# gdalsanto/flamo

Hardware: AMD Instinct MI355X
Metric: freq-bin*channel products/sec (fwd+bwd), nfft=96000 8x8ch (higher is better)
Workload: dtype f32; 1 GPU; BASELINE configs[1]: Shell(FFT -> Series(Matrix 8x8, GEQ 8x8) -> iFFT), nfft=96000, batch 32 per GPU, fwd+bwd of (y**2).mean(), parameter grads; nfft=96000, channels=8, batch_per_gpu=32, parallelism=dp1 (batch), input_grad=False

## Files before the change

flamo_amd/_lib.py:

```python
from __future__ import annotations

import ctypes as C
import os
import subprocess
import threading

_HERE = os.path.dirname(os.path.abspath(__file__))
LIB_PATH = os.environ.get("FLAMO_HIP_LIB") or os.path.join(_HERE, "libflamo_hip.so")
CSRC = os.path.join(_HERE, "csrc")

_lock = threading.Lock()
_lib = None

_vp, _i, _l, _d, _sz = C.c_void_p, C.c_int, C.c_long, C.c_double, C.c_size_t

_SIGNATURES = {
    "fl_version": (_i, []),
    "fl_last_error": (C.c_char_p, []),
    "fl_twiddle_fill_f32": (_i, [_vp, _i, _vp]),
    "fl_twiddle_fill_f64": (_i, [_vp, _i, _vp]),
    "fl_fft_plan": (_i, [_i, _i, C.POINTER(_i), C.POINTER(_i)]),
    "fl_fft_scratch_elems": (_sz, [_i, _i, _i]),
    "fl_debug_set_fft_max_single": (_i, [_i]),
    "fl_debug_set_fft_fast": (_i, [_i]),
    "fl_rfft_f32": (_i, [_vp, _l, _i, _vp, _l, _vp, _vp, _i, _i, _d, _d, _i, _vp]),
    "fl_rfft_f64": (_i, [_vp, _l, _i, _vp, _l, _vp, _vp, _i, _i, _d, _d, _i, _vp]),
    "fl_rfft_ci_f32": (_i, [_vp, _i, _i, _vp, _l, _vp, _vp, _i, _i, _d, _d, _i, _vp]),
    "fl_rfft_ci_f64": (_i, [_vp, _i, _i, _vp, _l, _vp, _vp, _i, _i, _d, _d, _i, _vp]),
    "fl_irfft_f32": (_i, [_vp, _l, _vp, _l, _i, _vp, _vp, _i, _i, _d, _d, _i, _vp]),
    "fl_irfft_f64": (_i, [_vp, _l, _vp, _l, _i, _vp, _vp, _i, _i, _d, _d, _i, _vp]),
    "fl_transpose": (_i, [_vp, _vp, _i, _i, _i, _l, _i, _vp]),
    "fl_spec_plan": (_i, [_i, C.POINTER(_i), C.POINTER(_i)]),
    "fl_spec_supports": (_i, [_i, _i, _i]),
    "fl_spec_supports_f64": (_i, [_i, _i, _i]),
    "fl_spec_aux_elems": (_sz, [_i]),
    "fl_spec_aux_fill_f32": (_i, [_vp, _i, _vp]),
    "fl_spec_aux_fill_f64": (_i, [_vp, _i, _vp]),
    "fl_debug_set_spec": (_i, [_i, _i]),
    "fl_debug_set_spec_times": (_i, [_vp]),
    "fl_spec_cols_fwd_f32": (_i, [_vp, _i, _i, _i, _vp, _vp, _i, _d, _vp]),
    "fl_spec_cols_fwd_f64": (_i, [_vp, _i, _i, _i, _vp, _vp, _i, _d, _vp]),
    "fl_spec_gradh_loop_supports_f32": (_i, [_i, _i, _i]),
    "fl_spec_gradh_loop_supports_f64": (_i, [_i, _i, _i]),
    "fl_spec_gradh_loop_f32": (_i, [_vp, _vp, _l, _l, _vp, _l, _l, _vp, _i, _i, _i, _i, _d, _i, _d, _vp, _vp]),
    "fl_spec_gradh_loop_f64": (_i, [_vp, _vp, _l, _l, _vp, _l, _l, _vp, _i, _i, _i, _i, _d, _i, _d, _vp, _vp]),
    "fl_spec_mid_f32": (_i, [_vp, _vp, _vp, _l, _l, _vp, _l, _l, _i, _vp, _i, _i, _i, _i, _d, _i, _i, _vp]),
    "fl_spec_mid_f64": (_i, [_vp, _vp, _vp, _l, _l, _vp, _l, _l, _i, _vp, _i, _i, _i, _i, _d, _i, _i, _vp]),
    "fl_spec_walk_supports": (_i, [_i, _i, _i]),
    "fl_spec_walk_spectrum_elems": (_sz, [_i, _i, _i]),
    "fl_spec_walk_workgroups": (_i, [_i, _i]),
    "fl_spec_walk_partition": (_i, [_i, _i, _i, C.POINTER(_i)]),
    "fl_spec_mid_walk_f32": (_i, [_vp, _vp, _vp, _vp, _l, _l, _i, _vp, _i, _i, _i, _i, _d, _i, _i, _vp, _vp]),
    "fl_spec_gradh_slices": (_i, [_i, _i]),
    "fl_spec_gradh_walk_f32": (_i, [_vp, _vp, _vp, _l, _l, _l, _i, _vp, _i, _i, _i, _i, _d, _i, _vp, _vp]),
    "fl_sum_parts_c64": (_i, [_vp, _l, _i, _vp, _l, _vp]),
    "fl_debug_set_walk": (_i, [_i, _i, _i, _vp]),
    "fl_debug_set_walk_stamps": (_i, [_vp]),
    "fl_wall_clock_khz": (_i, []),
    "fl_spec_cols_inv_f32": (_i, [_vp, _vp, _i, _i, _i, _i, _vp, _i, _d, _d, _vp, _vp, _vp, _vp]),
    "fl_spec_cols_blocks_f32": (_i, [_i, _i, _i]),
    "fl_spec_cols_blocks_f64": (_i, [_i, _i, _i]),
    "fl_spec_cols_inv_inplace_ok_f32": (_i, [_i, _i]),
    "fl_spec_cols_inv_inplace_ok_f64": (_i, [_i, _i]),
    "fl_spec_cols_inv_grad_supported_f32": (_i, [_i, _i]),
    "fl_spec_cols_inv_grad_supported_f64": (_i, [_i, _i]),
    "fl_mean_square_final_f32": (_i, [_vp, _i, _d, _vp, _vp]),
    "fl_mean_square_final_f64": (_i, [_vp, _i, _d, _vp, _vp]),
    "fl_pack_toggle": (_i, [_vp, _i, _vp, _vp, _vp, _vp]),
    "fl_spec_cols_inv_f64": (_i, [_vp, _vp, _i, _i, _i, _i, _vp, _i, _d, _d, _vp, _vp, _vp, _vp]),
    "fl_permute_bins_c64": (_i, [_vp, _l, _vp, _l, _i, _i, _i, _vp]),
    "fl_permute_bins_c128": (_i, [_vp, _l, _vp, _l, _i, _i, _i, _vp]),
    "fl_mimo_c64": (_i, [_vp, _l, _l, _l, _i, _vp, _l, _l, _l, _vp, _l, _l, _l, _i, _i, _i, _i, _i, _vp]),
    "fl_mimo_c128": (_i, [_vp, _l, _l, _l, _i, _vp, _l, _l, _l, _vp, _l, _l, _l, _i, _i, _i, _i, _i, _vp]),
    "fl_mimo_diag_c64": (_i, [_vp, _l, _l, _i, _vp, _l, _l, _l, _vp, _l, _l, _l, _i, _i, _i, _i, _vp]),
    "fl_mimo_diag_c128": (_i, [_vp, _l, _l, _i, _vp, _l, _l, _l, _vp, _l, _l, _l, _i, _i, _i, _i, _vp]),
    "fl_mimo_gradh_c64": (_i, [_vp, _l, _l, _l, _vp, _l, _l, _l, _vp, _l, _d, _i, _i, _i, _i, _i, _vp]),
    "fl_mimo_gradh_c128": (_i, [_vp, _l, _l, _l, _vp, _l, _l, _l, _vp, _l, _d, _i, _i, _i, _i, _i, _vp]),
    "fl_mimo_gradh_scaled_c64": (_i, [_vp, _l, _l, _l, _vp, _l, _l, _l, _vp, _l, _d, _vp, _i, _i, _i, _i, _i, _vp]),
    "fl_mimo_gradh_scaled_c128": (_i, [_vp, _l, _l, _l, _vp, _l, _l, _l, _vp, _l, _d, _vp, _i, _i, _i, _i, _i, _vp]),
    "fl_mimo_gradh_diag_c64": (_i, [_vp, _l, _l, _l, _vp, _l, _l, _l, _vp, _l, _i, _i, _i, _i, _vp]),
    "fl_mimo_gradh_diag_c128": (_i, [_vp, _l, _l, _l, _vp, _l, _l, _l, _vp, _l, _i, _i, _i, _i, _vp]),
    "fl_mimo_gradw_blocks": (_i, [_i]),
    "fl_debug_set_mimo_variant": (_i, [_i, _i]),
    "fl_mimo_gradw_c64": (_i, [_vp, _l, _l, _l, _vp, _l, _l, _l, _vp, _vp, _i, _i, _i, _i, _i, _vp]),
    "fl_mimo_gradw_c128": (_i, [_vp, _l, _l, _l, _vp, _l, _l, _l, _vp, _vp, _i, _i, _i, _i, _i, _vp]),
    "fl_mimo_gradw_re_c64": (_i, [_vp, _l, _l, _l, _vp, _l, _l, _l, _vp, _vp, _i, _i, _i, _i, _i, _vp]),
    "fl_mimo_gradw_re_c128": (_i, [_vp, _l, _l, _l, _vp, _l, _l, _l, _vp, _vp, _i, _i, _i, _i, _i, _vp]),
    "fl_delay_response_c64": (_i, [_vp, _vp, _i, _vp, _i, _i, _i, _vp, _l, _vp]),
    "fl_delay_response_c128": (_i, [_vp, _vp, _i, _vp, _i, _i, _i, _vp, _l, _vp]),
    "fl_sos_response_c64": (_i, [_vp, _vp, _i, _i, _d, _vp, _i, _i, _i, _vp, _l, _vp]),
    "fl_sos_response_f32eval_c64": (_i, [_vp, _vp, _i, _i, _d, _vp, _i, _i, _i, _vp, _l, _vp]),
    "fl_sos_response_c128": (_i, [_vp, _vp, _i, _i, _d, _vp, _i, _i, _i, _vp, _l, _vp]),
    "fl_sos_bwd_blocks": (_i, [_i, _i, _i, _i]),
    "fl_debug_set_sos_chunk": (_i, [_i]),
    "fl_debug_set_rc_fast": (_i, [_i]),
    "fl_sos_response_bwd_c64": (_i, [_vp, _l, _vp, _l, _vp, _vp, _i, _i, _d, _vp, _i, _i, _i, _vp, _vp]),
    "fl_sos_response_bwd_c128": (_i, [_vp, _l, _vp, _l, _vp, _vp, _i, _i, _d, _vp, _i, _i, _i, _vp, _vp]),
    "fl_sos_response_apply_max_ni": (_i, [_i]),
    "fl_sos_response_apply_c64": (_i, [_vp, _vp, _i, _i, _i, _vp, _l, _l, _i, _d, _vp, _i, _i, _i, _vp, _l, _vp, _l, _l, _vp]),
    "fl_sos_response_bwd_outer_c64": (_i, [_vp, _l, _l, _vp, _l, _l, _i, _i, _i, _vp, _l, _vp, _vp, _i, _d, _vp, _i, _i, _i, _vp, _vp]),
    "fl_sos_response_rc_c64": (_i, [_vp, _vp, _i, _i, _i, _i, _vp, _d, _vp, _i, _i, _i, _vp, _l, _vp, _l, _i, _vp]),
    "fl_geq_response_c64": (_i, [_vp, _i, _i, _vp, _vp, _vp, _i, _d, _vp, _i, _i, _i, _vp, _l, _i, _vp]),
    "fl_geq_response_rc_c64": (_i, [_vp, _i, _i, _vp, _vp, _vp, _i, _i, _i, _vp, _d, _vp, _i, _i, _i, _vp, _l, _vp, _l, _i, _vp]),
    "fl_sos_response_bwd_rc_c64": (_i, [_vp, _l, _vp, _l, _vp, _vp, _i, _i, _i, _i, _vp, _d, _vp, _i, _i, _i, _vp, _vp, _vp]),
    "fl_geq_sections": (_i, [_vp, _i, _i, _i, _vp, _vp, _vp, _vp]),
    "fl_geq_sections_bwd": (_i, [_vp, _i, _vp, _vp, _l, _i, _i, _i, _vp, _vp, _vp]),
    "fl_geq_sections_bwd_w": (_i, [_vp, _i, _vp, _vp, _l, _i, _i, _i, _vp, _vp, _vp, _i, _i, _vp, _vp]),
    "fl_geq_sections_bwd_w64": (_i, [_vp, _i, _vp, _vp, _l, _i, _i, _i, _vp, _vp, _vp, _i, _i, _vp, _vp]),
    "fl_sos_response_rc_c128": (_i, [_vp, _vp, _i, _i, _i, _i, _vp, _d, _vp, _i, _i, _i, _vp, _l, _vp, _l, _vp]),
    "fl_geq_response_rc_c128": (_i, [_vp, _i, _i, _vp, _vp, _vp, _i, _i, _i, _vp, _d, _vp, _i, _i, _i, _vp, _l, _vp, _l, _vp]),
    "fl_sos_response_bwd_rc_c128": (_i, [_vp, _l, _vp, _l, _vp, _vp, _i, _i, _i, _i, _vp, _d, _vp, _i, _i, _i, _vp, _vp, _vp]),
    "fl_geq_bwd_lanes_blocks": (_i, [_i, _i, _i, _i, _i, _i, _i, _i]),
    "fl_geq_bwd_lanes_wrows": (_i, [_i, _i, _i, _i, _i, _i, _i]),
    "fl_geq_response_bwd_lanes_c64": (_i, [_i, _vp, _l, _vp, _l, _vp, _vp, _i, _i, _i, _i, _vp, _d, _vp, _i, _i, _i, _vp, _vp, _vp, _vp]),
    "fl_geq_sections_bwd_lanes": (_i, [_vp, _i, _vp, _vp, _i, _vp, _vp, _d, _i, _i, _vp, _vp, _vp, _i, _i, _vp, _vp]),
    "fl_geq_bwd_lanes_blocks_f64": (_i, [_i, _i, _i, _i, _i, _i, _i, _i]),
    "fl_geq_bwd_lanes_wrows_f64": (_i, [_i, _i, _i, _i, _i, _i, _i]),
    "fl_geq_response_bwd_lanes_c128": (_i, [_i, _vp, _l, _vp, _l, _vp, _vp, _i, _i, _i, _i, _vp, _d, _vp, _i, _i, _i, _vp, _vp, _vp, _vp]),
    "fl_geq_sections_bwd_lanes_f64": (_i, [_vp, _i, _vp, _vp, _i, _vp, _vp, _d, _i, _i, _vp, _vp, _vp, _i, _i, _vp, _vp]),
    "fl_debug_set_cascade_lanes": (_i, [_i, _i, _i]),
    "fl_debug_set_cascade_stamps": (_i, [_vp, _i]),
    "fl_solve_max_n": (_i, [_i]),
    "fl_solve_ws_max_n": (_i, []),
    "fl_solve_ws_bytes": (_l, [_i, _i, _i]),
    "fl_solve_ws_c64": (_i, [_vp, _l, _i, _i, _vp, _l, _l, _l, _vp, _l, _l, _l, _i, _i, _i, _i, _vp, _l, _vp]),
    "fl_solve_ws_c128": (_i, [_vp, _l, _i, _i, _vp, _l, _l, _l, _vp, _l, _l, _l, _i, _i, _i, _i, _vp, _l, _vp]),
    "fl_solve_c64": (_i, [_vp, _l, _i, _i, _vp, _l, _l, _l, _vp, _l, _l, _l, _i, _i, _i, _i, _vp]),
    "fl_solve_c128": (_i, [_vp, _l, _i, _i, _vp, _l, _l, _l, _vp, _l, _l, _l, _i, _i, _i, _i, _vp]),
    "fl_solve_scaled_c64": (_i, [_vp, _l, _vp, _l, _i, _vp, _l, _l, _l, _vp, _l, _l, _l, _i, _i, _i, _i, _vp]),
    "fl_solve_scaled_c128": (_i, [_vp, _l, _vp, _l, _i, _vp, _l, _l, _l, _vp, _l, _l, _l, _i, _i, _i, _i, _vp]),
    "fl_solve_kept_lu_elems": (_sz, [_i, _i, _i]),
    "fl_solve_kept_piv_elems": (_sz, [_i, _i, _i]),
    "fl_solve_scaled_keep_c64": (_i, [_vp, _l, _vp, _l, _vp, _l, _l, _l, _vp, _l, _l, _l, _i, _i, _i, _i, _vp, _vp, _vp]),
    "fl_solve_scaled_keep_c128": (_i, [_vp, _l, _vp, _l, _vp, _l, _l, _l, _vp, _l, _l, _l, _i, _i, _i, _i, _vp, _vp, _vp]),
    "fl_solve_kept_adjoint_c64": (_i, [_vp, _vp, _vp, _l, _l, _l, _vp, _l, _l, _l, _i, _i, _i, _i, _vp]),
    "fl_solve_kept_adjoint_c128": (_i, [_vp, _vp, _vp, _l, _l, _l, _vp, _l, _l, _l, _i, _i, _i, _i, _vp]),
    "fl_solve_fdn_keep_tile": (_i, [_i, _i]),
    "fl_solve_fdn_wadj_supported": (_i, [_i]),
    "fl_solve_dud2_grads_w_c64": (_i, [_vp, _l, _l, _vp, _l, _l, _vp, _vp, _l, _l, _vp, _l, _vp, _l, _vp, _l, _l, _l, _i, _i, _i, _vp, _l, _vp, _l,
                                       _vp, _vp, _vp, _vp, _l, _vp, _l, _vp, _vp]),
    "fl_solve_dud2_grads_w_c128": (_i, [_vp, _l, _l, _vp, _l, _l, _vp, _vp, _l, _l, _vp, _l, _vp, _l, _vp, _l, _l, _l, _i, _i, _i, _vp, _l, _vp, _l,
                                       _vp, _vp, _vp, _vp, _l, _vp, _l, _vp, _vp]),
    "fl_solve_fdn_wadj_c64": (_i, [_vp, _l, _l, _vp, _l, _l, _vp, _vp, _l, _l, _vp, _i, _vp, _l, _vp, _i, _vp, _l, _vp, _l, _l, _l, _i, _i, _i, _vp, _l, _vp]),
    "fl_solve_fdn_wadj_c128": (_i, [_vp, _l, _l, _vp, _l, _l, _vp, _vp, _l, _l, _vp, _i, _vp, _l, _vp, _i, _vp, _l, _vp, _l, _l, _l, _i, _i, _i, _vp, _l, _vp]),
    "fl_solve_fdn_keep_c64": (_i, [_vp, _l, _l, _vp, _l, _l, _vp, _vp, _l, _l, _vp, _i, _vp, _l, _vp, _i, _vp, _l, _vp, _l, _l, _l, _i, _i, _i, _vp, _vp, _vp]),
    "fl_solve_fdn_keep_c128": (_i, [_vp, _l, _l, _vp, _l, _l, _vp, _vp, _l, _l, _vp, _i, _vp, _l, _vp, _i, _vp, _l, _vp, _l, _l, _l, _i, _i, _i, _vp, _vp, _vp]),
    "fl_solve_kept_adjoint_rank1_c64": (_i, [_vp, _vp, _i, _vp, _i, _vp, _l, _vp, _l, _l, _l, _i, _i, _i, _vp]),
    "fl_solve_kept_adjoint_rank1_c128": (_i, [_vp, _vp, _i, _vp, _i, _vp, _l, _vp, _l, _l, _l, _i, _i, _i, _vp]),
    "fl_solve_dud_c64": (_i, [_vp, _l, _l, _vp, _vp, _l, _l, _i, _vp, _l, _l, _l, _vp, _l, _l, _l, _i, _i, _i, _i, _vp]),
    "fl_solve_dud_c128": (_i, [_vp, _l, _l, _vp, _vp, _l, _l, _i, _vp, _l, _l, _l, _vp, _l, _l, _l, _i, _i, _i, _i, _vp]),
    "fl_solve_dud_grads_blocks": (_i, [_i, _i]),
    "fl_solve_fdn_c64": (_i, [_vp, _l, _l, _vp, _l, _l, _vp, _vp, _l, _l, _i, _vp, _i, _vp, _l, _vp, _i, _vp, _l, _vp, _l, _l, _l, _i, _i, _i, _vp]),
    "fl_solve_fdn_c128": (_i, [_vp, _l, _l, _vp, _l, _l, _vp, _vp, _l, _l, _i, _vp, _i, _vp, _l, _vp, _i, _vp, _l, _vp, _l, _l, _l, _i, _i, _i, _vp]),
    "fl_solve_dud2_c64": (_i, [_vp, _l, _l, _vp, _l, _l, _i, _vp, _vp, _l, _l, _i, _vp, _l, _l, _l, _vp, _l, _l, _l, _i, _i, _i, _i, _vp]),
    "fl_solve_dud2_c128": (_i, [_vp, _l, _l, _vp, _l, _l, _i, _vp, _vp, _l, _l, _i, _vp, _l, _l, _l, _vp, _l, _l, _l, _i, _i, _i, _i, _vp]),
    "fl_solve_dud2_grads_c64": (_i, [_vp, _l, _l, _vp, _l, _l, _vp, _vp, _l, _l, _vp, _vp, _l, _l, _l, _i, _i, _i, _i, _vp, _l, _vp, _l, _vp, _vp, _vp, _vp, _l, _vp, _l, _vp, _vp]),
    "fl_solve_dud2_grads_c128": (_i, [_vp, _l, _l, _vp, _l, _l, _vp, _vp, _l, _l, _vp, _vp, _l, _l, _l, _i, _i, _i, _i, _vp, _l, _vp, _l, _vp, _vp, _vp, _vp, _l, _vp, _l, _vp, _vp]),
    "fl_solve_dud_grads_c64": (_i, [_vp, _l, _l, _vp, _vp, _l, _l, _vp, _vp, _l, _l, _l, _i, _i, _i, _i, _vp, _l, _vp, _l, _vp, _vp, _vp]),
    "fl_solve_dud_grads_c128": (_i, [_vp, _l, _l, _vp, _vp, _l, _l, _vp, _vp, _l, _l, _l, _i, _i, _i, _i, _vp, _l, _vp, _l, _vp, _vp, _vp]),
    "fl_debug_set_solve_variant": (_i, [_i]),
    "fl_mean_square_scratch_bytes": (_sz, []),
    "fl_mean_square_f32": (_i, [_vp, _l, _l, _l, _vp, _vp, _vp]),
    "fl_mean_square_f64": (_i, [_vp, _l, _l, _l, _vp, _vp, _vp]),
    "fl_mean_square_bwd_f32": (_i, [_vp, _vp, _vp, _l, _l, _l, _vp]),
    "fl_mean_square_bwd_f64": (_i, [_vp, _vp, _vp, _l, _l, _l, _vp]),
    "fl_cabs_c64": (_i, [_vp, _vp, _l, _l, _l, _l, _vp]),
    "fl_cabs_c128": (_i, [_vp, _vp, _l, _l, _l, _l, _vp]),
    "fl_cabs_bwd_c64": (_i, [_vp, _vp, _vp, _l, _l, _l, _l, _vp]),
    "fl_cabs_bwd_c128": (_i, [_vp, _vp, _vp, _l, _l, _l, _l, _vp]),
    "fl_sparsity_f32": (_i, [_vp, _i, _i, _vp, _vp]),
    "fl_sparsity_f64": (_i, [_vp, _i, _i, _vp, _vp]),
    "fl_sparsity_bwd_f32": (_i, [_vp, _vp, _i, _i, _vp, _vp]),
    "fl_sparsity_bwd_f64": (_i, [_vp, _vp, _i, _i, _vp, _vp]),
    "fl_mse_f32": (_i, [_vp, _vp, _l, _i, _vp, _vp, _vp]),
    "fl_mse_f64": (_i, [_vp, _vp, _l, _i, _vp, _vp, _vp]),
    "fl_mse_bwd_f32": (_i, [_vp, _vp, _vp, _vp, _l, _i, _vp]),
    "fl_mse_bwd_f64": (_i, [_vp, _vp, _vp, _vp, _l, _i, _vp]),
    "fl_matrix_exp_stash_elems": (_sz, [_i]),
    "fl_debug_set_expm_mfma": (_i, [_i]),
    "fl_matrix_exp_f32": (_i, [_vp, _i, _i, _vp, _vp, _vp]),
    "fl_matrix_exp_f64": (_i, [_vp, _i, _i, _vp, _vp, _vp]),
    "fl_matrix_exp_bwd_f32": (_i, [_vp, _i, _i, _vp, _vp, _vp]),
    "fl_matrix_exp_bwd_f64": (_i, [_vp, _i, _i, _vp, _vp, _vp]),
    "fl_matrix_exp_cplx_f32": (_i, [_vp, _i, _i, _vp, _vp, _vp]),
    "fl_matrix_exp_cplx_f64": (_i, [_vp, _i, _i, _vp, _vp, _vp]),
    "fl_matrix_exp_bwd_cplx_f32": (_i, [_vp, _i, _i, _vp, _vp, _vp]),
    "fl_matrix_exp_bwd_cplx_f64": (_i, [_vp, _i, _i, _vp, _vp, _vp]),
    "fl_matrix_exp_both_f32": (_i, [_vp, _i, _i, _vp, _vp, _vp, _vp]),
    "fl_matrix_exp_both_f64": (_i, [_vp, _i, _i, _vp, _vp, _vp, _vp]),
    "fl_matrix_exp_bwd_both_f32": (_i, [_vp, _vp, _i, _i, _vp, _vp, _vp]),
    "fl_matrix_exp_bwd_both_f64": (_i, [_vp, _vp, _i, _i, _vp, _vp, _vp]),
    "fl_eig_c64": (_i, [_vp, _l, _i, _i, _vp, _l, _vp, _l, _vp, _vp]),
    "fl_eig_c128": (_i, [_vp, _l, _i, _i, _vp, _l, _vp, _l, _vp, _vp]),
    "fl_launch_pair_begin": (_i, []),
    "fl_launch_pair_pending": (_i, []),
    "fl_debug_launch_pair_count": (_l, []),
    "fl_debug_set_pair_stamps": (_i, [_vp]),
# ... 50 lines not shown
```

flamo_amd/csrc/cascade2.hip:

```cpp
#include "common.h"
#include "response_common.h"
#include "rc_ba_body.h"
#include "fusedfwd.h"

namespace fl {

typedef double d2 __attribute__((ext_vector_type(2)));
typedef double d4 __attribute__((ext_vector_type(4)));
template <typename T> struct Vec;
template <> struct Vec<float> { typedef f2 v2; typedef f4 v4; };
template <> struct Vec<double> { typedef d2 v2; typedef d4 v4; };
__device__ __forceinline__ float rcp_of(float x) { return __builtin_amdgcn_rcpf(x); }
__device__ __forceinline__ double rcp_of(double x) {
    double r = __builtin_amdgcn_rcp(x);
    r = fma(r, fma(-x, r, 1.0), r);
    return fma(r, fma(-x, r, 1.0), r);
}

template <typename T>
struct LanesArgs {
    const double* b;
    const double* a;
    int S, C;
    double g;
    const cx<double>* Wd;
    int nfft, bin0, m_local;
    const cx<T>* gH;
    long g_pitch;
    const cx<T>* G;
    long h_pitch;
    const T* Wr;
    T* psum;
    T* pq;
    T* partW;
    const cx<T>* oG;
    const cx<T>* oX;
    long o_gb, o_gn, o_xb, o_xn;
    int oB;
    int npb, rows, seff, s_first, tb, tbp, ntiles, tph, half, L1, nlow, tiles_low, nbx;
    int lds1;
    long long* stamps;
    int skip;
    unsigned pol;
};

template <int NSUM, typename P2, typename T>
__device__ __forceinline__ void lane_bin(P2 C0, P2 C1, P2 C2, P2 x, T uu, P2 qa, P2 qb, P2& t0, P2& t1, P2& t2) {
    const P2 R = C1 * x.x + C0;
    const P2 I = C2 * x.y;
    P2 n = R * R;
    n = I * I + n;
    const T r = rcp_of(n.x * n.y);
    const P2 inv = P2{n.y, n.x} * r;
    const P2 uR = R * inv, uI = I * inv;
    t0 = uR * qa.x + t0;
    t0 = uI * qa.y + t0;
    t2 = uR * qb.x + t2;
    t2 = uI * qb.y + t2;
    if constexpr (NSUM == 3) {
        const P2 uq = qa * uu;
        t1 = uR * uq.x + t1;
        t1 = uI * uq.y + t1;
    }
}

template <typename RT, int NIW, int PPR, int NSUM, bool OUTER>
__global__ void __launch_bounds__(sizeof(RT) == 8 ? 384 : 768, sizeof(RT) == 8 ? 2 : 3) sos_bwd_lanes_kernel(const LanesArgs<RT> A) {
    typedef typename Vec<RT>::v2 P2;
    typedef typename Vec<RT>::v4 P4;
    typedef cx<RT> cT;
    extern __shared__ __attribute__((aligned(32))) char smem[];
    const int t = threadIdx.x, lane = t & 63, wave = t >> 6;
    const int bx = blockIdx.x, cg = blockIdx.y;
    const int npb = A.npb, tbp = A.tbp, S = A.S, C = A.C;
    struct Bufs {
        P4* qs;
        P2* xs;
        RT* us;
    };
    auto bufs_at = [&](int which) {
        Bufs B;
        char* p = smem + (size_t)which * A.lds1;
        B.qs = reinterpret_cast<P4*>(p);
        B.xs = reinterpret_cast<P2*>(B.qs + (size_t)npb * tbp);
        B.us = reinterpret_cast<RT*>(B.xs + tbp);
        return B;
    };

    const int nl = npb * A.seff;
    const bool l_on = t < nl;
    const int sl = A.s_first + (l_on ? t / npb : 0), pl = l_on ? t % npb : 0;
    const int c = cg * npb + pl;
    P2 C0lo = {(RT)1.0, (RT)1.0}, C1lo = {(RT)0.0, (RT)0.0}, C0hi = {(RT)1.0, (RT)1.0}, C2 = {(RT)0.0, (RT)0.0};
    if (l_on) {
        const double g2 = A.g * A.g;
        const double b0 = A.b[(size_t)sl * C + c], b1 = A.b[(size_t)(S + sl) * C + c], b2 = A.b[(size_t)(2 * S + sl) * C + c];
        const double a0 = A.a[(size_t)sl * C + c], a1 = A.a[(size_t)(S + sl) * C + c], a2 = A.a[(size_t)(2 * S + sl) * C + c];
        const double SB = b0 + g2 * b2, TB = A.g * b1, DB = b0 - g2 * b2;
        const double SA = a0 + g2 * a2, TA = A.g * a1, DA = a0 - g2 * a2;
        C0lo = P2{(RT)(SB + TB), (RT)(SA + TA)};
        C1lo = P2{(RT)(-SB), (RT)(-SA)};
        C0hi = P2{(RT)(TB - SB), (RT)(TA - SA)};
        C2 = P2{(RT)DB, (RT)DA};
    }
    const bool wave_on = wave * 64 < nl;

    P2 acc0 = {(RT)0.0, (RT)0.0}, acc1 = {(RT)0.0, (RT)0.0}, acc2 = {(RT)0.0, (RT)0.0};
    struct Tile {
        int f0, n, kbase, kstep;
        bool low;
    };
    auto tile_of = [&](int tile) {
        Tile T;
        if (A.bin0 < 0) {
            if (tile == A.ntiles - 1) {
                T.f0 = A.nfft >> 1; T.n = 1; T.low = false; T.kbase = A.nfft >> 1; T.kstep = 0;
            } else {
                const int hr = tile / A.tph, sub = tile - hr * A.tph;
                T.f0 = hr * A.half + sub * A.tb;
                T.n = A.tb;
                T.low = (hr & 1) == 0;
                T.kbase = (hr >> 1) + A.L1 * ((hr & 1) * A.half + sub * A.tb);
                T.kstep = A.L1;
            }
        } else {
            if (tile < A.tiles_low) {
                T.f0 = tile * A.tb; T.n = min(A.tb, A.nlow - T.f0); T.low = true;
            } else {
                T.f0 = A.nlow + (tile - A.tiles_low) * A.tb; T.n = min(A.tb, A.m_local - T.f0); T.low = false;
            }
            T.kbase = A.bin0 + T.f0;
            T.kstep = 1;
        }
        return T;
    };

    constexpr bool RC = NIW > 0 && !OUTER;
    constexpr int JPT = RC ? ((NIW >= 16 || sizeof(RT) == 8) ? 1 : (PPR >= 2 ? 2 : PPR)) : (OUTER ? PPR : 1);
    constexpr int JG = (RC || OUTER) ? PPR / JPT : 1;
    constexpr int NG = OUTER ? 2 : (NIW > 0 ? NIW : 1);
    constexpr int TRIPS = (RC || OUTER) ? 1 : 4;
    struct Item {
        cT gv[NG];
        cT hv[JPT];
        cx<double> w1;
    };
    Item pre[TRIPS];
    const int nitems = A.tb * A.rows * JG;
    int it_i[TRIPS], it_r[TRIPS], it_j[TRIPS];
#pragma unroll
    for (int q = 0; q < TRIPS; ++q) {
        const int it = t + q * (int)blockDim.x;
        const int ir = it / JG;
        it_j[q] = (it - ir * JG) * JPT;
        it_i[q] = ir % A.tb;
        it_r[q] = it < nitems ? ir / A.tb : -1;
    }
    constexpr int NWJ = RC ? JPT : 1, NWN = RC ? NIW : 1;
    RT wrow[NWJ][NWN];
    P2 aw[NWJ][NWN];
#pragma unroll
    for (int j = 0; j < NWJ; ++j)
#pragma unroll
        for (int nn = 0; nn < NWN; ++nn) {
            wrow[j][nn] = RC ? A.Wr[(it_j[0] + j) * NIW + nn] : (RT)0.0;
            aw[j][nn] = P2{(RT)0.0, (RT)0.0};
        }
    auto at = [](const cT* base, unsigned byte_off) {
        return *reinterpret_cast<const cT*>(reinterpret_cast<const char*>(base) + byte_off);
    };
    auto at_nt = [](const cT* base, unsigned byte_off) {
        typedef RT rv2 __attribute__((ext_vector_type(2)));
        const rv2 v = __builtin_nontemporal_load(reinterpret_cast<const rv2*>(reinterpret_cast<const char*>(base) + byte_off));
        return cT(v.x, v.y);
    };
    auto request = [&](const Tile& T) {
        const int np = (T.n + 1) & ~1;
#pragma unroll
        for (int q = 0; q < TRIPS; ++q) {
            const int i = it_i[q], r = it_r[q];
            if (r < 0 || i >= np) continue;
            const int ii = i < T.n ? i : T.n - 1;
            const int f = T.f0 + ii, k = T.kbase + ii * T.kstep;
            pre[q].w1 = A.Wd[k];
            const int row = cg * A.rows + r;
            if constexpr (OUTER) {
#pragma unroll
                for (int bb = 0; bb < 2; ++bb)
                    pre[q].gv[bb] = bb < A.oB ? A.oG[(size_t)bb * A.o_gb + (size_t)row * A.o_gn + f] : cT((RT)0.0, (RT)0.0);
                const unsigned hoff = (unsigned)(((size_t)(row * PPR) * A.h_pitch + f) * sizeof(cT));
#pragma unroll
                for (int j = 0; j < JPT; ++j) pre[q].hv[j] = at(A.G + (size_t)j * A.h_pitch, hoff);
            } else if constexpr (RC) {
                const unsigned goff = (unsigned)(((size_t)(row * NIW) * A.g_pitch + f) * sizeof(cT));
                const unsigned hoff = (unsigned)(((size_t)(row * PPR + it_j[q]) * A.h_pitch + f) * sizeof(cT));
                if (A.pol & POL_LANES_GH_NT) {
#pragma unroll
                    for (int nn = 0; nn < NG; ++nn) pre[q].gv[nn] = at_nt(A.gH + (size_t)nn * A.g_pitch, goff);
                } else {
#pragma unroll
                    for (int nn = 0; nn < NG; ++nn) pre[q].gv[nn] = at(A.gH + (size_t)nn * A.g_pitch, goff);
                }
                if (A.pol & POL_LANES_G_NT) {
#pragma unroll
                    for (int j = 0; j < JPT; ++j) pre[q].hv[j] = at_nt(A.G + (size_t)j * A.h_pitch, hoff);
                } else {
#pragma unroll
                    for (int j = 0; j < JPT; ++j) pre[q].hv[j] = at(A.G + (size_t)j * A.h_pitch, hoff);
                }
            } else {
                pre[q].gv[0] = A.gH[(size_t)row * A.g_pitch + f];
                pre[q].hv[0] = A.G[(size_t)row * A.h_pitch + f];
            }
        }
    };
    RT qsum[TRIPS][JPT];
#pragma unroll
    for (int q = 0; q < TRIPS; ++q)
#pragma unroll
        for (int j = 0; j < JPT; ++j) qsum[q][j] = (RT)0.0;
    auto bin_work = [&](const Tile& T, const Bufs& B) {
        const int n = T.n, np = (n + 1) & ~1;
#pragma unroll
        for (int q = 0; q < TRIPS; ++q) {
            const int i = it_i[q], r = it_r[q], j0 = it_j[q];
            if (r < 0 || i >= np) continue;
            const bool valid = i < n;
            const Item& P = pre[q];
            const RT sn = (RT)(-P.w1.y);
            if (r == 0 && j0 == 0) {
                B.xs[i] = P2{(RT)(T.low ? 1.0 - P.w1.x : 1.0 + P.w1.x), sn};
                if constexpr (NSUM == 3) B.us[i] = (RT)(1.0 - P.w1.x);
            }
            if constexpr (RC) {
#pragma unroll
                for (int j = 0; j < JPT; ++j) {
                    P2 gi = {(RT)0.0, (RT)0.0};
#pragma unroll
                    for (int nn = 0; nn < NIW; ++nn) gi = P2{P.gv[nn].x, P.gv[nn].y} * wrow[j][nn] + gi;
                    const cT h = valid ? P.hv[j] : cT((RT)0.0, (RT)0.0);
                    const bool live = valid && !(h.x == eps_of<RT>() && h.y == (RT)0.0);
                    const cT qv(gi.x * h.x + gi.y * h.y, gi.x * h.y - gi.y * h.x);
                    const cT qz = live ? qv : cT((RT)0.0, (RT)0.0);
                    B.qs[(size_t)(r * PPR + j0 + j) * tbp + i] = P4{qz.x, qz.y, sn * qz.y, -(sn * qz.x)};
                    qsum[q][j] += qz.x;
#pragma unroll
                    for (int nn = 0; nn < NIW; ++nn) aw[j][nn] = P2{h.x, h.y} * P2{P.gv[nn].x, P.gv[nn].y} + aw[j][nn];
                }
            } else if constexpr (OUTER) {
                const int f = T.f0 + (valid ? i : n - 1);
#pragma unroll 4
                for (int j = 0; j < PPR; ++j) {
                    cT gi((RT)0.0, (RT)0.0);
                    for (int bb = 0; bb < A.oB && bb < 2; ++bb) fma_cxc(gi, P.gv[bb], A.oX[(size_t)bb * A.o_xb + (size_t)j * A.o_xn + f]);
                    const cT h = P.hv[j];
                    const bool live = valid && !(h.x == eps_of<RT>() && h.y == (RT)0.0);
                    const cT qv(gi.x * h.x + gi.y * h.y, gi.x * h.y - gi.y * h.x);
                    const cT qz = live ? qv : cT((RT)0.0, (RT)0.0);
                    B.qs[(size_t)(r * PPR + j) * tbp + i] = P4{qz.x, qz.y, sn * qz.y, -(sn * qz.x)};
                    qsum[q][j] += qz.x;
                }
            } else {
                const cT gi = P.gv[0], h = P.hv[0];
                const bool live = valid && !(h.x == eps_of<RT>() && h.y == (RT)0.0);
                const cT qv(gi.x * h.x + gi.y * h.y, gi.x * h.y - gi.y * h.x);
                const cT qz = live ? qv : cT((RT)0.0, (RT)0.0);
                B.qs[(size_t)r * tbp + i] = P4{qz.x, qz.y, sn * qz.y, -(sn * qz.x)};
                qsum[q][0] += qz.x;
            }
        }
    };

    const int t_begin = (int)((long)bx * A.ntiles / A.nbx), t_end = (int)((long)(bx + 1) * A.ntiles / A.nbx);
    long long st[6] = {0, 0, 0, 0, 0, 0};
    const long long k_start = A.stamps ? (long long)__builtin_readcyclecounter() : 0;
    const long long r_start = A.stamps ? (long long)__builtin_amdgcn_s_memrealtime() : 0;
#define FL_STAMP(slot, t_prev)                                                  \
    if (A.stamps) {                                                             \
        const long long now_ = (long long)__builtin_readcyclecounter();         \
        st[slot] += now_ - t_prev;                                              \
        t_prev = now_;                                                          \
    }
    Tile T = tile_of(t_begin < t_end ? t_begin : 0), Tn = T;
    if (t_begin < t_end) {
        request(T);
        bin_work(T, bufs_at(0));
        if (t_begin + 1 < t_end) {
            Tn = tile_of(t_begin + 1);
            request(Tn);
        }
    }
    __syncthreads();
    for (int tile = t_begin; tile < t_end; ++tile) {
        long long tp = A.stamps ? (long long)__builtin_readcyclecounter() : 0;
        const Bufs B = bufs_at((tile - t_begin) & 1);
        const int np = (T.n + 1) & ~1;
        const bool low = T.low;
        auto section_work = [&]() {
            if (!(wave_on && !(A.skip & 2))) return;
            const P2 C0 = low ? C0lo : C0hi, C1 = low ? C1lo : -C1lo;
            P2 t0 = {(RT)0.0, (RT)0.0}, t1 = {(RT)0.0, (RT)0.0}, t2 = {(RT)0.0, (RT)0.0};
            const P4* qrow = B.qs + (size_t)pl * tbp;
#pragma unroll 2
            for (int i = 0; i < np; i += 2) {
                P4 x4;
                if constexpr (sizeof(RT) == 4) {
                    x4 = *reinterpret_cast<const P4*>(B.xs + i);
                } else {
                    const P2 xa = B.xs[i], xb = B.xs[i + 1];
                    x4 = P4{xa.x, xa.y, xb.x, xb.y};
                }
                const P4 qA = qrow[i], qB = qrow[i + 1];
                RT u0 = (RT)0.0, u1 = (RT)0.0;
                if constexpr (NSUM == 3) {
                    const P2 u2 = *reinterpret_cast<const P2*>(B.us + i);
                    u0 = u2.x;
                    u1 = u2.y;
// ... 281 lines not shown
        const int L2 = -bin0;
        P.half = L2 / 2;
        P.L1 = (nfft / 2) / L2;
        int best = 0;
        double best_score = -1;
        for (int d = 8; d <= 64 && d <= P.half && d <= tb_max; ++d) {
            if (P.half % d) continue;
            if (g_lanes_tb > 0 && d != g_lanes_tb) continue;
            const long nt = 2L * P.L1 * (P.half / d) + 1;
            const long nbx = nt < nbx_target ? nt : nbx_target;
            const long per = (nt + nbx - 1) / nbx;
            const double score = (double)nt / (double)(nbx * per) * d / (d + 6.0);
            if (score > best_score) {
                best_score = score;
                best = d;
            }
        }
        if (!best) return P;
        P.tb = best;
        P.tph = P.half / best;
        P.ntiles = 2 * P.L1 * P.tph + 1;
    } else {
        P.tb = g_lanes_tb > 0 ? g_lanes_tb : 32;
        if (P.tb > tb_max) P.tb = tb_max & ~1;
        const long q4 = ((long)nfft + 3) / 4;
        long nlow = q4 - bin0;
        if (nlow < 0) nlow = 0;
        if (nlow > m_local) nlow = m_local;
        P.nlow = (int)nlow;
        P.tiles_low = (P.nlow + P.tb - 1) / P.tb;
        P.ntiles = P.tiles_low + (m_local - P.nlow + P.tb - 1) / P.tb;
    }
    P.nbx = P.ntiles < nbx_target ? P.ntiles : nbx_target;
    const int npad = (P.tb + 1) & ~1;
    P.tbp = npad + 1;
    P.lds1 = ((size_t)P.npb * P.tbp * 16 + (size_t)(P.tbp + 1) * 8 + (size_t)((P.tbp + 3) & ~3) * 4) * sc;
    P.lds1 = (P.lds1 + 31) & ~(size_t)31;
    {
        const size_t items = mode == 0 ? (size_t)P.tb * P.rows : (size_t)P.threads;
        const size_t need = items * (mode == 1 ? jpt * (niw > 1 ? niw : 1) : jpt) * 4 * sc;
        if (2 * P.lds1 < need) P.lds1 = (need + 63) / 64 * 32;
    }
    if (2 * P.lds1 > device_lds_limit()) return P;
    if ((size_t)C * (size_t)m_local * 8 * sc >= (1ull << 32)) return P;
    P.ok = 1;
    return P;
}

template <typename T>
static void lanes_fill(LanesArgs<T>& A, const LanesPlan& P) {
    A.npb = P.npb; A.rows = P.rows; A.seff = P.seff; A.s_first = P.s_first; A.tb = P.tb; A.tbp = P.tbp; A.ntiles = P.ntiles;
    A.tph = P.tph; A.half = P.half; A.L1 = P.L1; A.nlow = P.nlow; A.tiles_low = P.tiles_low; A.nbx = P.nbx;
    A.lds1 = (int)P.lds1;
}

template <typename T>
static int lanes_sections_bwd_impl(const void* gain, int in_kind, const void* psum, const void* pq, int nbx, const void* b, const void* a,
                                   double gamma, int nb, int C, const void* consts, void* ggain, const void* partW, int wrows, int wn,
                                   void* gW, void* stream) {
    FL_REQUIRE(gain && psum && pq && b && a && consts && ggain, "geq_sections_bwd_lanes: null pointer");
    FL_REQUIRE(in_kind >= 0 && in_kind <= 4 && nb >= 4 && C > 0 && nbx > 0, "geq_sections_bwd_lanes: bad sizes");
    FL_REQUIRE(wn == 0 || (partW && gW && wrows > 0), "geq_sections_bwd_lanes: bad constant-factor partials");
    const int epb = nbx > 512 ? 1 : nbx > 256 ? 2 : 4;
    const int main_blocks = cdiv_i((long)nb * C, epb);
    hipLaunchKernelGGL(geq_bwd_lanes_kernel<T>, dim3(main_blocks + cdiv_i(wn, 4)), dim3(256), 0, (hipStream_t)stream, gain, in_kind,
                       (const T*)psum, (const T*)pq, nbx, (const double*)b, (const double*)a, gamma, nb, C,
                       (const double*)consts, ggain, main_blocks, epb, (const T*)partW, wrows, wn, (T*)gW);
    FL_CHECK_LAUNCH("geq_sections_bwd_lanes");
    return FL_OK;
}

}

using namespace fl;

extern "C" int fl_geq_bwd_lanes_blocks(int m_local, int C, int S, int nfft, int bin0, int ppr, int niw, int mode) {
    const LanesPlan P = lanes_plan(m_local, C, S, nfft, bin0, ppr, niw, mode);
    return P.ok ? P.nbx : 0;
}
extern "C" int fl_geq_bwd_lanes_wrows(int m_local, int C, int S, int nfft, int bin0, int ppr, int niw) {
    const LanesPlan P = lanes_plan(m_local, C, S, nfft, bin0, ppr, niw, 1);
    return P.ok ? P.nbx * P.ng : 0;
}
FL_ENTRY_C64_C128(fl_geq_response_bwd_lanes, (int mode, const void* gH, long g_pitch, const void* G, long h_pitch, const void* b, const void* a,
                                              int S, int No, int Nmid, int Ni, const void* Wr, double gamma, const void* Wd, int nfft,
                                              int bin0, int m_local, void* psum, void* pq, void* partW, void* stream),
                  (mode, gH, g_pitch, G, h_pitch, b, a, S, No, Nmid, Ni, Wr, gamma, Wd, nfft, bin0, m_local, psum, pq, partW, stream)) {
    FL_REQUIRE(mode == 0 || mode == 1, "geq_response_bwd_lanes: mode 0 (plain) or 1 (constant factor)");
    FL_REQUIRE(gH && G && b && a && Wd && psum && pq, "geq_response_bwd_lanes: null pointer");
    FL_REQUIRE(mode == 0 || (Wr && partW), "geq_response_bwd_lanes: the constant-factor mode needs Wr and partW");
    FL_REQUIRE(g_pitch >= m_local && h_pitch >= m_local, "geq_response_bwd_lanes: pitches must be >= m_local");
    const int C = No * Nmid, ppr = mode == 1 ? Nmid : 1;
    const LanesPlan P = lanes_plan(m_local, C, S, nfft, bin0, ppr, Ni, mode, (int)sizeof(T));
    if (!P.ok) {
        set_error("geq_response_bwd_lanes: unsupported shape (ask fl_geq_bwd_lanes_blocks first)");
        return FL_ERR_UNSUPPORTED;
    }
    LanesArgs<T> A{};
    A.b = (const double*)b; A.a = (const double*)a; A.S = S; A.C = C; A.g = gamma; A.Wd = (const cx<double>*)Wd;
    A.nfft = nfft; A.bin0 = bin0; A.m_local = m_local; A.gH = (const cx<T>*)gH; A.g_pitch = g_pitch;
    A.G = (const cx<T>*)G; A.h_pitch = h_pitch; A.Wr = (const T*)Wr; A.psum = (T*)psum; A.pq = (T*)pq;
    A.partW = (T*)partW;
    A.stamps = g_lanes_stamps;
    A.skip = g_lanes_skip;
    A.pol = stream_policy();
    lanes_fill(A, P);
    const dim3 grid(P.nbx, P.ng), block(P.threads);
    const size_t lds = 2 * P.lds1;
    int rc = FL_OK;
    dispatch<0, 8, 4, 2, 16>(mode == 0 ? 0 : Ni, [&](auto NIW) {
        constexpr int niw = decltype(NIW)::value;
        static bool done[kMaxDevices] = {};
        auto kern = sos_bwd_lanes_kernel<T, niw, niw ? niw : 1, 2, false>;
        rc = lanes_ensure_lds(reinterpret_cast<const void*>(kern), lds, done);
        if (rc == FL_OK) hipLaunchKernelGGL(kern, grid, block, lds, (hipStream_t)stream, A);
    });
    if (rc) return rc;
    FL_CHECK_LAUNCH("geq_response_bwd_lanes");
    return FL_OK;
}
extern "C" int fl_geq_sections_bwd_lanes(const void* gain, int in_kind, const void* psum, const void* pq, int nbx, const void* b, const void* a,
                                         double gamma, int nb, int C, const void* consts, void* ggain, const void* partW, int wrows, int wn,
                                         void* gW, void* stream) {
    return lanes_sections_bwd_impl<float>(gain, in_kind, psum, pq, nbx, b, a, gamma, nb, C, consts, ggain, partW, wrows, wn, gW, stream);
}
extern "C" int fl_geq_bwd_lanes_blocks_f64(int m_local, int C, int S, int nfft, int bin0, int ppr, int niw, int mode) {
    const LanesPlan P = lanes_plan(m_local, C, S, nfft, bin0, ppr, niw, mode, 8);
    return P.ok ? P.nbx : 0;
}
extern "C" int fl_geq_bwd_lanes_wrows_f64(int m_local, int C, int S, int nfft, int bin0, int ppr, int niw) {
    const LanesPlan P = lanes_plan(m_local, C, S, nfft, bin0, ppr, niw, 1, 8);
    return P.ok ? P.nbx * P.ng : 0;
}
extern "C" int fl_geq_sections_bwd_lanes_f64(const void* gain, int in_kind, const void* psum, const void* pq, int nbx, const void* b, const void* a,
                                             double gamma, int nb, int C, const void* consts, void* ggain, const void* partW, int wrows,
                                             int wn, void* gW, void* stream) {
    return lanes_sections_bwd_impl<double>(gain, in_kind, psum, pq, nbx, b, a, gamma, nb, C, consts, ggain, partW, wrows, wn, gW, stream);
}
extern "C" int fl_debug_set_cascade_lanes(int on, int blocks_per_cu, int tile_bins) {
    const int prev = g_lanes | ((g_lanes && !g_lanes_fwd) ? 2 : 0);
    if (on >= 0) {
        g_lanes = on & 1;
        g_lanes_fwd = (on & 1) && !(on & 2);
    }
    if (blocks_per_cu >= 0) g_lanes_bpc = blocks_per_cu;
    if (tile_bins >= 0) g_lanes_tb = tile_bins;
    return prev;
}
extern "C" int fl_debug_set_cascade_stamps(void* device_buffer, int skip) {
    g_lanes_stamps = (long long*)device_buffer;
    g_lanes_skip = skip;
    return 0;
}
```

flamo_amd/csrc/specwalk.hip:

```cpp
#include "spectral_common.h"

namespace fl {
using namespace sp32;

struct WalkArgs {
    const cf* S;
    cf* S2;
    const cf* H;
    long hs_m, hs_n;
    int conj_h;
    const cf* W;
    int n, L, L1, L2, Bn;
    float spec_scale;
    int spec_interior2;
    int pre_half;
    const int* bounds;
    cf* Xp;
    long long* dbg_times;
    unsigned pol;
    long long* stamps;
};

__device__ __forceinline__ int opaque(int v) {
    asm volatile("" : "+v"(v));
    return v;
}
__device__ __forceinline__ f2 lds_rd(unsigned byte_addr, int off) {
    f2 v;
    asm volatile("ds_read_b64 %0, %1 offset:%2" : "=v"(v) : "v"(byte_addr), "i"(off));
    return v;
}
template <int N>
__device__ __forceinline__ void lds_reads_done(f2 (&r)[N], cf (&v)[N]) {
    asm volatile("s_waitcnt lgkmcnt(0)" ::: "memory");
#pragma unroll
    for (int i = 0; i < N; ++i) {
        asm volatile("" : "+v"(r[i]));
        v[i] = c2(r[i]);
    }
}
#ifndef FL_XP_PAIRS
#define FL_XP_PAIRS 1
#endif
typedef float f4 __attribute__((ext_vector_type(4)));
__device__ __forceinline__ void st_nt16(cf* base, unsigned byte_off, f2 lo, f2 hi) {
    const f4 q = {lo.x, lo.y, hi.x, hi.y};
    __builtin_nontemporal_store(q, reinterpret_cast<f4*>(reinterpret_cast<char*>(base) + byte_off));
}

__device__ __forceinline__ void st_pl16(cf* base, unsigned byte_off, f2 lo, f2 hi) {
    const f4 q = {lo.x, lo.y, hi.x, hi.y};
    *reinterpret_cast<f4*>(reinterpret_cast<char*>(base) + byte_off) = q;
}

__device__ __forceinline__ f2 cj(f2 a) { return f2{a.x, -a.y}; }
__device__ __forceinline__ f2 rot_i(f2 a) { return f2{-a.y, a.x}; }
__device__ __forceinline__ f2 pfma(f2 a, f2 b, f2 c) { return __builtin_elementwise_fma(a, b, c); }
__device__ __forceinline__ f2 cmul2(f2 a, f2 b) { return pfma(f2{a.y, a.y}, rot_i(b), f2{a.x, a.x} * b); }
__device__ __forceinline__ f2 cmac2(f2 acc, f2 a, f2 b, f2 ib) { return pfma(f2{a.y, a.y}, ib, pfma(f2{a.x, a.x}, b, acc)); }

__device__ __forceinline__ f2 cmulc(f2 b, f2 a, f2 ia) { return pfma(f2{b.y, b.y}, ia, f2{b.x, b.x} * a); }
#if FL_PK_DEV
#define FL_PK_ADD(name, mods, plain)                                                 \
    __device__ __forceinline__ f2 name(f2 a, f2 b) {                                 \
        f2 r;                                                                        \
        asm("v_pk_add_f32 %0, %1, %2 " mods : "=v"(r) : "v"(a), "v"(b));             \
        return r;                                                                    \
    }
#else
#define FL_PK_ADD(name, mods, plain) \
    __device__ __forceinline__ f2 name(f2 a, f2 b) { return plain; }
#endif
FL_PK_ADD(add_pm, "neg_hi:[0,1]", (f2{a.x + b.x, a.y - b.y}))
FL_PK_ADD(add_mp, "neg_lo:[0,1]", (f2{a.x - b.x, a.y + b.y}))
FL_PK_ADD(add_cj, "neg_hi:[1,1]", (f2{a.x + b.x, -a.y - b.y}))
FL_PK_ADD(sub_cj, "neg_lo:[0,1] neg_hi:[1,0]", (f2{a.x - b.x, b.y - a.y}))
#undef FL_PK_ADD
__device__ __forceinline__ f2 fma_mi(f2 x, f2 g, f2 acc) {
#if FL_PK_DEV
    asm("v_pk_fma_f32 %0, %1, %2, %0 op_sel:[1,1,0] op_sel_hi:[1,0,1] neg_hi:[0,1,0]" : "+v"(acc) : "v"(x), "v"(g));
    return acc;
#else
    return f2{acc.x + x.y * g.y, acc.y - x.y * g.x};
// ... 261 lines not shown
#if FL_XP_PAIRS
                    cf* xo = a.Xp + ((size_t)u * 2 + grp) * (NI * LEN) + 2 * p;
                    if (a.pol & POL_WALK_XP_PLAIN) {
                        if (grp) {
#pragma unroll
                            for (int j = 0; j < NI / 2; ++j) st_pl16(xo, 16u * (unsigned)(j * LEN), xm[2 * j], xm[2 * j + 1]);
                        } else {
#pragma unroll
                            for (int j = 0; j < NI / 2; ++j) st_pl16(xo, 16u * (unsigned)(j * LEN), xk[2 * j], xk[2 * j + 1]);
                        }
                    } else if (grp) {
#pragma unroll
                        for (int j = 0; j < NI / 2; ++j) st_nt16(xo, 16u * (unsigned)(j * LEN), xm[2 * j], xm[2 * j + 1]);
                    } else {
#pragma unroll
                        for (int j = 0; j < NI / 2; ++j) st_nt16(xo, 16u * (unsigned)(j * LEN), xk[2 * j], xk[2 * j + 1]);
                    }
#else
                    cf* xo = a.Xp + ((size_t)u * 2 + grp) * (NI * LEN) + p;
                    if (grp) {
#pragma unroll
                        for (int nn = 0; nn < NI; ++nn) st_nt(xo, 8u * (unsigned)(nn * LEN), c2(xm[nn]));
                    } else {
#pragma unroll
                        for (int nn = 0; nn < NI; ++nn) st_nt(xo, 8u * (unsigned)(nn * LEN), c2(xk[nn]));
                    }
#endif
                }
                cf* zk_p = XI + yk_o + grp * MO * LENP;
                cf* zm_p = zm_dst + (twin ? grp * MO * LENP : 0);
#pragma unroll
                for (int m2 = 0; m2 < MO; ++m2) {
                    f2 ka_ = {0.f, 0.f}, kb_ = {0.f, 0.f}, ma_ = {0.f, 0.f}, mb_ = {0.f, 0.f};
#pragma unroll
                    for (int nn = 0; nn < NI; ++nn) {
                        ka_ = pfma(f2{h[0][m2][nn].x, h[0][m2][nn].x}, xk[nn], ka_);
                        kb_ = pfma(f2{h[0][m2][nn].y, h[0][m2][nn].y}, xk[nn], kb_);
                        ma_ = pfma(f2{h[1][m2][nn].x, h[1][m2][nn].x}, xm[nn], ma_);
                        mb_ = pfma(f2{h[1][m2][nn].y, h[1][m2][nn].y}, xm[nn], mb_);
                    }
                    const f2 yk = pk_add_i(ka_, kb_), ym = pk_add_i(ma_, mb_);
                    f2 zk, zm;
                    pre_pair(phv * yk, phv * ym, icw, nicw, zk, zm);
                    zk_p[m2 * LENP] = c2(zk);
                    zm_p[twin ? m2 * LENP : 0] = c2(zm);
                }
            }
            if (DBG) w_ph[0] += clock64() - t_last;
            lds_barrier();
            FL_STAMP(1)
            if (grp == 0) P4(selfm);
            else if (next) P1(selfm);
            if (DBG) w_ph[1] += clock64() - t_last;
            lds_barrier();
            FL_STAMP(2)
            if (grp == 0) P5(selfm, r, rm, u - r * a.Bn);
            else if (next) {
                if (u + 2 < u_hi) fetch(u + 2);
                P2(selfm);
            }
            if (DBG) w_ph[2] += clock64() - t_last;
            lds_barrier();
            FL_STAMP(3)
        }
    }
    if (a.stamps && tid == 0) {
        wait_vm0();
        a.stamps[2 * blockIdx.x + 1] = (long long)__builtin_amdgcn_s_memrealtime();
    }
    if (DBG && a.dbg_times && tid == 0) {
        long long* o = a.dbg_times + (size_t)blockIdx.x * 8;
        o[0] = t_begin;
        o[1] = clock64();
#pragma unroll
        for (int i = 0; i < 4; ++i) o[2 + i] = t_ph[i];
    }
    if (DBG && a.dbg_times && (tid == 0 || tid == 256))
        a.dbg_times[(size_t)blockIdx.x * 8 + 6 + grp] = grp == 0 && a.spec_interior2 == 7
            ? (q_ph[0] >> 4) | ((q_ph[1] >> 4) << 21) | ((q_ph[2] >> 4) << 42)
            : (w_ph[0] >> 4) | ((w_ph[1] >> 4) << 21) | ((w_ph[2] >> 4) << 42);
#undef FL_STAMP
}

struct GradhArgs {
    const cf* Sg;
    const cf* Xp;
    cf* dH;
    long ds_s, ds_m, ds_n;
    const cf* W;
    int n, L, L1, L2, Bn, NS;
    float scale_g;
    const float* out_scale;
    int interior2_g;
    long long* dbg_times;
    unsigned pol;
};

template <int A, int B, int NI, int NO, int NSC, int OCC, int DEPTH, bool DBG = false>
__global__ void __launch_bounds__(512, OCC) spec_gradh_walk(GradhArgs a) {
    extern __shared__ __attribute__((aligned(16))) char smem[];
    constexpr int LEN = A * B, LENP = walk_pitch(LEN);
    constexpr int NOL = NO / NSC;
    constexpr int UB = 2 * NOL * LENP;
    constexpr int NI1 = 2 * B * NOL, NI2 = 2 * NOL * A;
    constexpr int NW1 = (NI1 + 63) / 64;
    constexpr int SBG = NW1 * A * 64;
    constexpr int SBX = 8 * NI * 64;
    static_assert(LEN <= 256, "one bin pair per thread pair");
    static_assert(NO % NSC == 0 && NOL % 2 == 0 && NI % 2 == 0 && A % 2 == 0, "16-byte DMA granules");
    static_assert(NI1 <= 256 && NI2 <= 256, "an FFT stage of one unit fits one group");
    static_assert(DEPTH == 1 || DEPTH == 2, "one or two items in flight");
    constexpr int GA = A / 2, XA = NI / 2;
    constexpr int P2_OFF = 256 - ((NI2 + 63) / 64) * 64;
    cf* XF = reinterpret_cast<cf*>(smem);
    cf* Yb = XF + 2 * UB;
    cf* stage_g = Yb + UB;
    cf* stage_x = stage_g + DEPTH * SBG;
    constexpr int TWP = tw_pitch(A), TWL = (B * TWP + 1) & ~1;
    cf* tw = stage_x + DEPTH * SBX;
    cf* ws = tw + TWL;
    const int tid = threadIdx.x;
    const int wave = __builtin_amdgcn_readfirstlane(tid >> 6), lane = tid & 63;
    const int grp = wave >> 2;
    const int P = a.L1 / 2 + 1;
    const int xcd = blockIdx.x & 7, q_ = blockIdx.x >> 3;
    const int r = (q_ / (a.NS * NSC)) * 8 + xcd, sl = (q_ / NSC) % a.NS, mo = (q_ % NSC) * NOL;
    if (r >= P) return;
    const int rm = (a.L1 - r) % a.L1;
    const bool selfm = rm == r;
    const int b_lo = (int)((long)a.Bn * sl / a.NS), n_it = (int)((long)a.Bn * (sl + 1) / a.NS) - b_lo;
    const size_t bstride_g = (size_t)a.L1 * a.L2 * NO;
    const unsigned sg_lds = lds_addr_of(stage_g), sx_lds = lds_addr_of(stage_x);

    auto fetch_g = [&](int i, int cw) {
        const int b = b_lo + ((a.pol & POL_GRADH_FORWARD) ? i : n_it - 1 - i);
        const unsigned sg_buf = sg_lds + (unsigned)((i % DEPTH) * SBG * 8);
        const int hi = lane >> 5;
        int item0 = 64 * cw + 2 * (lane & 31);
        if (item0 >= NI1 || (item0 >= B * NOL && selfm)) item0 = 0;
        const int m0 = item0 % NOL, tb = (item0 / NOL) % B, slot = item0 / (NOL * B);
        const cf* src = a.Sg + (size_t)b * bstride_g + (size_t)(slot ? rm : r) * (a.L2 * NO) + ((hi * B + tb) * NO + mo + m0);
        if (a.pol & POL_GRADH_SG_NT) {
#pragma unroll
            for (int q = 0; q < A / 2; ++q) dma16p<true>(src + q * (2 * B * NO), sg_buf + (unsigned)(((cw * A + 2 * q) * 64) * 8));
        } else {
#pragma unroll
            for (int q = 0; q < A / 2; ++q) dma16p<false>(src + q * (2 * B * NO), sg_buf + (unsigned)(((cw * A + 2 * q) * 64) * 8));
        }
    };
    auto fetch_x = [&](int i, int cw) {
        const int b = b_lo + ((a.pol & POL_GRADH_FORWARD) ? i : n_it - 1 - i);
        const unsigned sx_buf = sx_lds + (unsigned)((i % DEPTH) * SBX * 8);
#if FL_XP_PAIRS
        int pp = 64 * (cw & 3) + lane;
        if (pp > LEN - 1) pp = LEN - 1;
        const cf* src = a.Xp + (((size_t)r * a.Bn + b) * 2 + (cw >> 2)) * (NI * LEN) + 2 * pp;
#else
        int pp = 64 * (cw & 3) + 2 * (lane & 31);
        if (pp > LEN - 2) pp = LEN - 2;
        const cf* src = a.Xp + (((size_t)r * a.Bn + b) * 2 + (cw >> 2)) * (NI * LEN) + (lane >> 5) * LEN + pp;
#endif
        if (a.pol & POL_GRADH_XP_NT) {
#pragma unroll
            for (int q = 0; q < NI / 2; ++q) dma16p<true>(src + q * (2 * LEN), sx_buf + (unsigned)(((cw * NI + 2 * q) * 64) * 8));
        } else {
#pragma unroll
            for (int q = 0; q < NI / 2; ++q) dma16p<false>(src + q * (2 * LEN), sx_buf + (unsigned)(((cw * NI + 2 * q) * 64) * 8));
        }
    };

    const int p = tid & 255;
    int slotB = 0, colB = 0;
    bool dc = false;
    const bool valid = p < LEN && pair_of(r, selfm, p, LEN, slotB, colB, dc);
    const int pc = p < LEN ? p : 0;
    f2 acc[NOL][NI];
#pragma unroll
    for (int m = 0; m < NOL; ++m)
#pragma unroll
        for (int nn = 0; nn < NI; ++nn) acc[m][nn] = f2{0.f, 0.f};
    const bool has_g = grp == 0 && (wave & 3) < NW1;
    const bool fetcher = DEPTH == 2 && wave >= 2 && wave <= 5;
    const int fi = wave - 2;
    const int xlo = NW1 >= 2 ? (fi == 0 ? 0 : fi == 1 ? 1 : fi == 2 ? 2 : 5) : (fi == 0 ? 0 : fi == 1 ? 1 : fi == 2 ? 3 : 6);
    const int xhi = NW1 >= 2 ? (fi == 0 ? 1 : fi == 1 ? 2 : fi == 2 ? 5 : 8) : (fi == 0 ? 1 : fi == 1 ? 3 : fi == 2 ? 6 : 8);
    int x_issued = 0;
    if (DEPTH == 2) {
        if (fetcher && fi < NW1 && n_it > 0) fetch_g(0, fi);
    } else if (has_g && n_it > 0) {
        fetch_g(0, wave & 3);
    }
    for (int j = tid; j < LEN; j += 512) {
        tw[(j / A) * TWP + j % A] = a.W[a.n + a.L1 + (j / A) * (j % A)];
        ws[j] = a.W[a.n + a.L1 + a.L2 + j];
    }
    const cf wr = a.W[r];
    lds_barrier();
    const f2 wk = v2(wr * ws[pc]);
    const f2 iws = grp ? rot_i(wk) : f2{wk.y, -wk.x}, niws = grp ? f2{-wk.x, -wk.y} : wk;
    const float hg = 0.5f * a.scale_g;
    const float sc = dc ? hg : hg * (a.interior2_g ? 2.f : 1.f);
    const f2 scv = grp ? f2{sc, -sc} : f2{sc, sc};
    const int yk_o = pc, ym_o = slotB * NOL * LENP + colB;

    long long g_ph[2] = {0, 0}, g_last = 0, g_begin = 0;
    if (DBG) g_begin = g_last = clock64();
#define FL_GSTAMP(i)                        \
    if (DBG) {                              \
        const long long t_now = clock64();  \
        g_ph[i] += t_now - g_last;          \
        g_last = t_now;                     \
    }
#pragma unroll 1
// ... 72 lines not shown
                }
            }
        } else if (t >= 1 && t <= n_it) {
            const int item = (opaque(tid) & 255) - P2_OFF;
            const int m = item % NOL, ka = (item / NOL) % A, slot = item / (NOL * A);
            if (item >= 0 && item < NI2 && !(slot && selfm)) {
                cf v[B];
                const cf* xr = XF + ((t - 1) & 1) * UB + (slot * NOL + m) * LENP + ka * B;
#pragma unroll
                for (int tb = 0; tb < B; ++tb) v[tb] = xr[tb];
                RegFFT<float, B, false>::run(v);
                cf* yr = Yb + (slot * NOL + m) * LENP + ka;
#pragma unroll
                for (int kb = 0; kb < B; ++kb) yr[A * kb] = v[kb];
            }
        }
        long long t_work = 0;
        if (DBG) t_work = clock64() - g_last;
        lds_barrier();
        FL_GSTAMP(1)
        if (DBG && a.dbg_times && lane == 0 && (wave == 0 || wave == 1 || wave == 4 || wave == 7))
            atomicAdd((unsigned long long*)(a.dbg_times + (size_t)blockIdx.x * 8 + (wave == 0 ? 4 : wave == 1 ? 5 : wave == 4 ? 6 : 7)), (unsigned long long)t_work);
    }
#undef FL_GSTAMP
    if (DBG && a.dbg_times && tid == 0) {
        long long* o = a.dbg_times + (size_t)blockIdx.x * 8;
        o[0] = g_begin;
        o[1] = clock64();
        o[2] = g_ph[0];
        o[3] = g_ph[1];
    }
    {
        const unsigned ik = (unsigned)r * LEN + p;
        const unsigned im = dc ? (unsigned)a.L : (unsigned)(slotB ? rm : r) * LEN + colB;
        if (valid && !(grp && im == ik)) {
            cf* out = a.dH + (size_t)sl * a.ds_s;
            const unsigned bin = grp ? im : ik;
            if (a.out_scale) {
                const float os = *a.out_scale;
#pragma unroll
                for (int m = 0; m < NOL; ++m)
#pragma unroll
                    for (int nn = 0; nn < NI; ++nn) acc[m][nn] *= os;
            }
#pragma unroll
            for (int m = 0; m < NOL; ++m) {
                unsigned o = 8u * ((unsigned)(mo + m) * (unsigned)a.ds_m + bin);
                const unsigned step = 8u * (unsigned)a.ds_n;
                if (a.pol & POL_GRADH_DH_NT) {
#pragma unroll
                    for (int nn = 0; nn < NI; ++nn) {
                        st_nt(out, o, c2(acc[m][nn]));
                        o += step;
                    }
                } else {
#pragma unroll
                    for (int nn = 0; nn < NI; ++nn) {
                        at(out, o) = c2(acc[m][nn]);
                        o += step;
                    }
                }
            }
        }
    }
}

__global__ void __launch_bounds__(256) sum_parts_kernel(const float4* __restrict__ parts, long stride4, int ns, float4* __restrict__ out, long n4) {
    const long j = (long)blockIdx.x * 256 + threadIdx.x;
    if (j >= n4) return;
    float4 s = parts[j];
    for (int k = 1; k < ns; ++k) {
        const float4 v = parts[(long)k * stride4 + j];
        s.x += v.x; s.y += v.y; s.z += v.z; s.w += v.w;
    }
    out[j] = s;
}

constexpr int kMaxWalkWgs = 1024;
static int g_walk = 1;
static int g_walk_wgs = 0;
static int g_walk_slices = 0;
static long long* g_walk_times = nullptr;
static long long* g_walk_stamps = nullptr;
static int g_walk_nsc = 2;
static int g_walk_fc = [] { const char* e = getenv("FLAMO_WALK_FC"); return e ? atoi(e) : 38; }();
static int g_walk_fc2 = [] { const char* e = getenv("FLAMO_WALK_FC2"); return e ? atoi(e) : 38; }();
static int g_walk_us = [] { const char* e = getenv("FLAMO_WALK_US"); return e ? atoi(e) : 16; }();

long long* walk_successor_stamp() { return g_walk_stamps ? g_walk_stamps + 2 * kMaxWalkWgs : nullptr; }

static long walk_wgs(int L1, int Bn) {
    const long units = (long)(L1 / 2 + 1) * Bn;
    long g = g_walk_wgs > 0 ? g_walk_wgs : device_cus();
    if (g > units) g = units;
    if (g >= 8) g -= g % 8;
    return g;
}

static int ensure_lds(const void* kern, size_t lds, bool* done ) {
    return ensure_dynamic_lds(kern, lds, false, done, "walking kernels");
}

template <int A, int B, int NI, int NO>
constexpr size_t walk_lds_bytes() {
    constexpr int LEN = A * B, LENP = walk_pitch(LEN), NCH = NI > NO ? NI : NO;
    return ((size_t)3 * 2 * NCH * LENP + 4 * A * 64 + ((B * tw_pitch(A) + 1) & ~1) + 3 * LEN + 64) * sizeof(cf);
}

template <int A, int B, int NI, int NO, int OCC>
static int launch_walk(const WalkArgs& a, hipStream_t st) {
    constexpr size_t lds = walk_lds_bytes<A, B, NI, NO>();
    static_assert(lds <= 160 * 1024, "LDS budget");
    static bool done[kMaxDevices] = {}, done_dbg[kMaxDevices] = {};
    auto kern = spec_mid_walk<A, B, NI, NO, OCC>;
    auto kern_dbg = spec_mid_walk<A, B, NI, NO, OCC, true>;
    int rc = ensure_lds(reinterpret_cast<const void*>(kern), lds, done);
    if (rc) return rc;
    if (a.dbg_times && (rc = ensure_lds(reinterpret_cast<const void*>(kern_dbg), lds, done_dbg))) return rc;
    const long g = walk_wgs(a.L1, a.Bn);
    if (a.dbg_times) hipLaunchKernelGGL(kern_dbg, dim3((unsigned)g), dim3(512), lds, st, a);
    else hipLaunchKernelGGL(kern, dim3((unsigned)g), dim3(512), lds, st, a);
    return FL_OK;
}

}

using namespace fl;

extern "C" {

int fl_debug_set_walk_stamps(void* buf) {
    g_walk_stamps = (long long*)buf;
    return FL_OK;
}

int fl_wall_clock_khz(void) {
    int dev = 0, khz = 0;
    if (hipGetDevice(&dev) != hipSuccess || hipDeviceGetAttribute(&khz, hipDeviceAttributeWallClockRate, dev) != hipSuccess || khz <= 0) khz = 100000;
    return khz;
}

int fl_debug_set_walk(int mode, int wgs, int slices, void* times) {
    g_walk_nsc = mode == 14 ? 4 : mode == 15 ? 1 : 2;
    g_walk = mode;
    g_walk_wgs = wgs;
    g_walk_slices = slices;
    g_walk_times = (long long*)times;
    return FL_OK;
}

static bool walk_shape(int l2, int n_in, int n_out) {
    auto ch = [](int c) { return c == 2 || c == 4 || c == 8; };
    return (l2 == 240 || l2 == 256) && ch(n_in) && ch(n_out);
}
int fl_spec_walk_supports(int nfft, int n_in, int n_out) {
    int l1, l2;
    if (!g_walk || spec_plan(nfft, l1, l2) != FL_OK) return 0;
    if (!walk_shape(l2, n_in, n_out)) return 0;
    return walk_lds_bytes<16, 16, 8, 8>() <= device_lds_limit();
}

int fl_spec_gradh_slices(int nfft, int Bn) {
    int l1, l2;
    if (spec_plan(nfft, l1, l2) != FL_OK || Bn <= 0) return 0;
    if (g_walk_slices > 0) return g_walk_slices < Bn ? g_walk_slices : Bn;
    const int P = l1 / 2 + 1;
    int ns = device_cus() / (2 * P);
    if (g_walk_nsc == 4) ns = 1;
    if (g_walk_nsc == 1) ns = device_cus() / P;
    if (ns < 1) ns = 1;
    return ns < Bn ? ns : Bn;
}

int fl_spec_gradh_walk_f32(const void* Sg, const void* Xp, void* dH_parts, long ds_s, long ds_m, long ds_n, int n_slices, const void* W,
                           int nfft, int Bn, int NI, int NO, double scale_g, int interior2_g, const void* out_scale, void* stream) {
    FL_REQUIRE(Sg && Xp && dH_parts && W, "spec_gradh_walk: null pointer");
    FL_REQUIRE(n_slices >= 1 && n_slices <= (Bn > 0 ? Bn : 1), "spec_gradh_walk: slices must be in [1, batch]");
    FL_REQUIRE(reinterpret_cast<uintptr_t>(Sg) % 16 == 0 && reinterpret_cast<uintptr_t>(Xp) % 16 == 0, "spec_gradh_walk: scratch arrays must be 16-byte aligned");
    if (Bn == 0) return FL_OK;
    GradhArgs a = {};
    int rc = spec_plan(nfft, a.L1, a.L2);
    if (rc) return rc;
    a.Sg = (const cf*)Sg; a.Xp = (const cf*)Xp; a.dH = (cf*)dH_parts; a.ds_s = ds_s; a.ds_m = ds_m; a.ds_n = ds_n;
    a.W = (const cf*)W; a.n = nfft; a.L = nfft / 2; a.Bn = Bn; a.NS = n_slices;
    a.scale_g = (float)scale_g; a.interior2_g = interior2_g; a.dbg_times = g_walk_times; a.out_scale = (const float*)out_scale;
    a.pol = stream_policy();
    FL_REQUIRE((size_t)NO * (size_t)ds_m * 8ull < (1ull << 32), "spec_gradh_walk: a partial plane set exceeds 32-bit offsets");
    const int P = a.L1 / 2 + 1;
    hipStream_t st = (hipStream_t)stream;
    int lrc = FL_ERR_UNSUPPORTED;
#define FL_GRADH(A_, B_, NI_, NO_, NSC_, OCC_, DEPTH_)                                                                            \
    {                                                                                                                            \
        constexpr int LEN = A_ * B_, LENP = walk_pitch(LEN), NOL = NO_ / NSC_;                                                   \
        constexpr size_t lds = ((size_t)3 * 2 * NOL * LENP + DEPTH_ * (((2 * B_ * NOL + 63) / 64) * A_ * 64 + 8 * NI_ * 64) +    \
                                ((B_ * tw_pitch(A_) + 1) & ~1) + LEN) * sizeof(cf);                                              \
        static_assert(lds <= 160 * 1024, "LDS budget");                                                                          \
        const unsigned nblk = (unsigned)(cdiv_i(P, 8) * 8 * n_slices * NSC_);                                                    \
        auto kern = spec_gradh_walk<A_, B_, NI_, NO_, NSC_, OCC_, DEPTH_>;                                                       \
        auto kern_dbg = spec_gradh_walk<A_, B_, NI_, NO_, NSC_, OCC_, DEPTH_, true>;                                             \
        static bool done[kMaxDevices] = {}, done_dbg[kMaxDevices] = {};                                                          \
        lrc = ensure_lds(reinterpret_cast<const void*>(kern), lds, done);                                                        \
        if (!lrc && a.dbg_times) lrc = ensure_lds(reinterpret_cast<const void*>(kern_dbg), lds, done_dbg);                       \
        if (!lrc) {                                                                                                              \
            if (a.dbg_times) hipLaunchKernelGGL(kern_dbg, dim3(nblk), dim3(512), lds, st, a);                                    \
            else hipLaunchKernelGGL(kern, dim3(nblk), dim3(512), lds, st, a);                                                    \
        }                                                                                                                        \
    }
#define FL_GRADH_ROWS(A_, B_)                                                                                                    \
    if (NI == 8 && NO == 8) {                                                                                                    \
        if (A_ == 16 && B_ == 15 && g_walk_nsc == 4) FL_GRADH(16, 15, 8, 8, 4, 4, 1)                                             \
        else if (A_ == 16 && B_ == 15 && g_walk_nsc == 1) FL_GRADH(16, 15, 8, 8, 1, 2, 1)                                        \
        else if (A_ == 16 && B_ == 15 && g_walk == 17) FL_GRADH(16, 15, 8, 8, 2, 2, 1)                                           \
        else FL_GRADH(A_, B_, 8, 8, 2, 2, 2)                                                                                     \
    }                                                                                                                            \
    else if (NI == 4 && NO == 8) FL_GRADH(A_, B_, 4, 8, 2, 2, 1)                                                                 \
    else if (NI == 2 && NO == 8) FL_GRADH(A_, B_, 2, 8, 2, 2, 1)                                                                 \
    else if (NI == 8 && NO == 4) FL_GRADH(A_, B_, 8, 4, 2, 2, 1)                                                                 \
    else if (NI == 4 && NO == 4) FL_GRADH(A_, B_, 4, 4, 2, 2, 1)                                                                 \
    else if (NI == 2 && NO == 4) FL_GRADH(A_, B_, 2, 4, 2, 2, 1)                                                                 \
    else if (NI == 8 && NO == 2) FL_GRADH(A_, B_, 8, 2, 1, 2, 1)                                                                 \
    else if (NI == 4 && NO == 2) FL_GRADH(A_, B_, 4, 2, 1, 2, 1)                                                                 \
    else if (NI == 2 && NO == 2) FL_GRADH(A_, B_, 2, 2, 1, 2, 1)
    if (a.L2 == 240) { FL_GRADH_ROWS(16, 15) }
    else if (a.L2 == 256) { FL_GRADH_ROWS(16, 16) }
#undef FL_GRADH_ROWS
#undef FL_GRADH
    if (lrc == FL_ERR_UNSUPPORTED && !walk_shape(a.L2, NI, NO)) {
        set_error("spec_gradh_walk: no kernel for nfft=%d, %d -> %d channels", nfft, NI, NO);
        return FL_ERR_UNSUPPORTED;
    }
    if (lrc) return lrc;
    FL_CHECK_LAUNCH("spec_gradh_walk");
    return FL_OK;
}

int fl_sum_parts_c64(const void* parts, long part_stride, int n_parts, void* out, long n, void* stream) {
    FL_REQUIRE(parts && out && n_parts >= 1 && n >= 0, "sum_parts: bad arguments");
    FL_REQUIRE(n % 2 == 0 && part_stride % 2 == 0 && reinterpret_cast<uintptr_t>(parts) % 16 == 0 && reinterpret_cast<uintptr_t>(out) % 16 == 0,
               "sum_parts: 16-byte granularity");
    if (n == 0) return FL_OK;
    const long n4 = n / 2;
    hipLaunchKernelGGL(sum_parts_kernel, dim3((unsigned)((n4 + 255) / 256)), dim3(256), 0, (hipStream_t)stream, (const float4*)parts,
                       part_stride / 2, n_parts, (float4*)out, n4);
    FL_CHECK_LAUNCH("sum_parts");
    return FL_OK;
}

int fl_spec_walk_workgroups(int nfft, int Bn) {
    int l1, l2;
    if (spec_plan(nfft, l1, l2) != FL_OK || Bn <= 0) return 0;
    return (int)walk_wgs(l1, Bn);
}

int fl_spec_walk_partition(int nfft, int Bn, int n_wg, int* bounds) {
    FL_REQUIRE(bounds && n_wg > 0 && Bn > 0, "spec_walk_partition: bad arguments");
    int L1, L2;
    int rc = spec_plan(nfft, L1, L2);
    if (rc) return rc;
    const int P = L1 / 2 + 1, U = P * Bn, UC = 20, US = g_walk_us, FC = g_walk_fc, FC2 = g_walk_fc2;
    auto ucost = [&](int u) { const int r = u / Bn; return (r == 0 || 2 * r == L1) ? US : UC; };
    auto sweep = [&](long cap, int* out) {
        int n = 0, u = 0;
        while (u < U) {
            if (out) out[n] = u;
            ++n;
            long c = FC + ucost(u);
            int last_r = u / Bn;
            ++u;
            while (u < U) {
                const int r = u / Bn;
                const long add = ucost(u) + (r != last_r ? FC2 : 0);
                if (c + add > cap) break;
                c += add;
                last_r = r;
                ++u;
            }
        }
        return n;
    };
    long lo = FC + UC, hi = (long)U * UC + (long)P * FC;
    while (lo < hi) {
        const long mid = (lo + hi) / 2;
        if (sweep(mid, nullptr) <= n_wg) hi = mid;
        else lo = mid + 1;
    }
    const int used = sweep(lo, bounds);
    for (int i = used; i <= n_wg; ++i) bounds[i] = U;
    return FL_OK;
}

size_t fl_spec_walk_spectrum_elems(int nfft, int Bn, int NI) {
    int l1, l2;
    if (spec_plan(nfft, l1, l2) != FL_OK || Bn < 0) return 0;
    return (size_t)(l1 / 2 + 1) * Bn * 2 * NI * l2;
}

int fl_spec_mid_walk_f32(const void* S, void* S2, void* Xp, const void* H, long hs_m, long hs_n, int conj_h, const void* W, int nfft, int Bn,
                         int NI, int NO, double spec_scale, int spec_interior2, int pre_half, const void* bounds, void* stream) {
    FL_REQUIRE(S && S2 && H && W, "spec_mid_walk: null pointer");
    FL_REQUIRE(S != S2, "spec_mid_walk: not an in-place kernel (the rows of a round are read while earlier rounds' are stored)");
    if (Bn == 0) return FL_OK;
    WalkArgs a = {};
    int rc = spec_plan(nfft, a.L1, a.L2);
    if (rc) return rc;
    a.S = (const cf*)S; a.S2 = (cf*)S2; a.H = (const cf*)H; a.hs_m = hs_m; a.hs_n = hs_n; a.conj_h = conj_h;
    a.W = (const cf*)W; a.n = nfft; a.L = nfft / 2; a.Bn = Bn;
    a.spec_scale = (float)spec_scale; a.spec_interior2 = spec_interior2; a.pre_half = pre_half; a.dbg_times = g_walk_times;
    a.Xp = (cf*)Xp;
    a.bounds = (const int*)bounds;
    a.pol = stream_policy();
    a.stamps = walk_wgs(a.L1, Bn) <= kMaxWalkWgs ? g_walk_stamps : nullptr;
    FL_REQUIRE((size_t)a.L1 * a.L2 * (NI > NO ? NI : NO) * 8ull < (1ull << 32), "spec_mid_walk: a batch item exceeds 32-bit offsets");
    FL_REQUIRE(reinterpret_cast<uintptr_t>(S) % 16 == 0, "spec_mid_walk: S must be 16-byte aligned");
    hipStream_t st = (hipStream_t)stream;
    rc = FL_ERR_UNSUPPORTED;
#define FL_WALK_ROWS(A_, B_)                                                  \
// ... 23 lines not shown
```

flamo_amd/ops.py:

```python
from __future__ import annotations

import ctypes
import math
import threading
from collections import namedtuple
from typing import NamedTuple, Optional, Tuple

import torch

from . import _lib

__all__ = ["rfft", "irfft", "spectral_apply", "permute_bins", "mimo", "solve", "delay_response", "sos_response", "geq_sections", "solve_dud", "to_planar", "set_bin_shard",
           "bin_shard"]


def _require_gpu(*ts: torch.Tensor) -> torch.device:
    dev = None
    for t in ts:
        if t is None:
            continue
        if not t.is_cuda:
            raise RuntimeError(
                "flamo_amd: tensors must live on a ROCm device (got %s); the HIP path has no CPU fallback" % t.device
            )
# ... 759 lines not shown
    if INVERSE_IN_PLACE and t_len == t_out == nfft and S2.numel() == B * (nfft // 2) * G and S2.is_contiguous() and \
            _fn("fl_spec_cols_inv_inplace_ok", real)(nfft, G):
        y = torch.empty(0, dtype=real, device=dev).set_(S2.untyped_storage(), 2 * S2.storage_offset(), (B, t_len, G))
    else:
        y = alloc((B, t_len, G), dtype=real, device=dev)
    if dev_scale is not None and (dev_scale.dtype != real or not dev_scale.is_cuda or dev_scale.numel() != 1):
        raise ValueError("spec_cols_inv: dev_scale must be one device scalar of the signal's dtype")
    parts = Sg = None
    if want_sumsq:
        nblk = int(_fn("fl_spec_cols_blocks", real)(nfft, B, G))
        parts = torch.empty(max(nblk, 1), dtype=torch.float64, device=dev)
    if grad_cols:
        assert want_sumsq and t_len == t_out == nfft and env_log2 == 0.0
        n_sg = B * (nfft // 2) * G
        Sg = sg_buf if sg_buf is not None and sg_buf.numel() == n_sg and sg_buf.dtype == S2.dtype and sg_buf.data_ptr() != S2.data_ptr() \
            else torch.empty(n_sg, dtype=S2.dtype, device=dev)
    with kernel_timer.span("spec_cols_inv+grad_cols" if grad_cols else "spec_cols_inv"):
        _lib.check(_fn("fl_spec_cols_inv", real)(S2.data_ptr(), y.data_ptr(), B, t_len, t_out, G, twiddles(nfft, real, dev).data_ptr(),
                                                 nfft, scale, env_log2, _ptr(parts), _ptr(dev_scale), _ptr(Sg), _stream()), "spec_cols_inv")
    if grad_cols:
        return y, parts, Sg
    return (y, parts) if want_sumsq else y


_WALK_MIN_BATCH = 4


def _walk_applies(nfft: int, B: int, NI: int, NO: int) -> bool:
    return B >= _WALK_MIN_BATCH and bool(_lib.lib().fl_spec_walk_supports(int(nfft), int(NI), int(NO)))


_walk_bounds = {}


def _walk_partition(nfft: int, B: int, dev: torch.device) -> torch.Tensor:
    L = _lib.lib()
    n_wg = int(L.fl_spec_walk_workgroups(nfft, B))
    key = (int(nfft), int(B), n_wg, dev.index if dev.index is not None else torch.cuda.current_device())
    t = _walk_bounds.get(key)
    if t is None:
        host = (ctypes.c_int * (n_wg + 1))()
        _lib.check(L.fl_spec_walk_partition(nfft, B, n_wg, host), "spec_walk_partition")
        if torch.cuda.is_current_stream_capturing():
            return None
        t = torch.tensor(list(host), dtype=torch.int32).to(dev)
        torch.cuda.current_stream(dev).synchronize()
        _walk_bounds[key] = t
    return t


def _spec_mid_walk(S, B, NI, NO, nfft, Hrm, conj_t, want_spec, spec_scale, interior2, pre_half):
    dev = S.device
    L = _lib.lib()
    bounds = _walk_partition(nfft, B, dev)
    S2 = torch.empty(B * (nfft // 2) * NO, dtype=torch.complex64, device=dev)
    Xp = torch.empty(int(L.fl_spec_walk_spectrum_elems(nfft, B, NI)), dtype=torch.complex64, device=dev) if want_spec else None
    hs_m, hs_n = _h_strides(Hrm, conj_t)
    tag = f"spec_mid_walk[{NI}->{NO}" + (",spec" if want_spec else "") + "]"
    with kernel_timer.span(tag):
        _lib.check(L.fl_spec_mid_walk_f32(S.data_ptr(), S2.data_ptr(), _ptr(Xp), Hrm.data_ptr(), hs_m, hs_n,
                                          int(bool(conj_t)), twiddles(nfft, torch.float32, dev).data_ptr(), nfft, B, NI, NO, spec_scale,
                                          int(interior2), int(pre_half), _ptr(bounds), _stream()), "spec_mid_walk")
    return S2, Xp


INVERSE_IN_PLACE = True
GRADH_LOOP = True
GRADH_LOOP_MAX_BATCH = 4


def _spec_gradh_loop(Sg, Xs, B, NI, NO, nfft, scale_g, host_factor=1.0, out_scale=None):
    dev = Sg.device
    M = nfft // 2 + 1
    real = _rdtype(Sg)
    P = _pitch(M)
    dH = _empty_rows((NO, NI), M, Sg.dtype, dev)
    with kernel_timer.span("spec_gradh_loop"):
        _lib.check(_fn("fl_spec_gradh_loop", real)(Sg.data_ptr(), Xs.data_ptr(), NI * P, P, dH.data_ptr(), NI * P, P,
                                                   twiddles(nfft, real, dev).data_ptr(), nfft, B, NI, NO, float(scale_g), 1,
                                                   float(host_factor), _ptr(out_scale), _stream()), "spec_gradh_loop")
    return dH.movedim(-1, 0)


def _spec_gradh_walk(Sg, Xp, B, NI, NO, nfft, scale_g, out_scale=None):
    dev = Sg.device
    L = _lib.lib()
    M = nfft // 2 + 1
    P = _pitch(M)
    ns = int(L.fl_spec_gradh_slices(nfft, B))
    parts = torch.empty((ns, NO, NI, P), dtype=torch.complex64, device=dev)
    with kernel_timer.span("spec_gradh_walk"):
        _lib.check(L.fl_spec_gradh_walk_f32(Sg.data_ptr(), Xp.data_ptr(), parts.data_ptr(), NO * NI * P, NI * P, P, ns,
                                            twiddles(nfft, torch.float32, dev).data_ptr(), nfft, B, NI, NO, scale_g, 1,
                                            _ptr(out_scale), _stream()), "spec_gradh_walk")
    if ns == 1:
        out = parts[0]
    else:
        out = torch.empty((NO, NI, P), dtype=torch.complex64, device=dev)
        with kernel_timer.span("sum_parts"):
            _lib.check(L.fl_sum_parts_c64(parts.data_ptr(), NO * NI * P, ns, out.data_ptr(), NO * NI * P, _stream()), "sum_parts")
    return out[..., :M].movedim(-1, 0)


class _SpecCfg(NamedTuple):
    nfft: int
    scale_f: float
    env_f: float
    scale_i: float
    env_i: float
    T: int
    NI: int
    NO: int
    route: str


def _spec_route(real, nfft, B, NI, NO) -> str:
    return "walk" if real == torch.float32 and _walk_applies(nfft, B, NI, NO) else "rows"


def _spec_backward_route(cfg, real, B, need_x, need_h) -> str:
    if cfg.route == "walk":
        return "walk"
    if need_h and not need_x and GRADH_LOOP and B <= GRADH_LOOP_MAX_BATCH and _fn("fl_spec_gradh_loop_supports", real)(cfg.nfft, cfg.NI, cfg.NO):
        return "loop"
    return "layered"


_SpectralTag = namedtuple("_SpectralTag", "x Hrm Hp Xs cfg parts version Sg")


class _SpectralApply(torch.autograd.Function):
    @staticmethod
    def forward(ctx, x, Hrm, nfft, scale_f, env_f, scale_i, env_i):
        _require_gpu(x, Hrm)
        if x.dtype not in (torch.float32, torch.float64) or x.dim() != 3:
            raise TypeError("spectral_apply expects a real float32 / float64 (B, T, N) signal")
        M = nfft // 2 + 1
        if Hrm.dim() != 3 or Hrm.shape[0] != M or Hrm.dtype != _cdtype(x.dtype):
            raise ValueError(f"spectral_apply: the response must be {_cdtype(x.dtype)} ({M}, N_out, N_in)")
        NO, NI = Hrm.shape[1], Hrm.shape[2]
        if x.shape[2] != NI:
            raise ValueError(f"response expects {NI} input channels, signal has {x.shape[2]}")
        xc = x.contiguous()
        if xc.data_ptr() % (2 * xc.element_size()):
            xc = xc.clone()
        Hp = _h_planar(Hrm.resolve_conj(), True)
        B, T = xc.shape[0], xc.shape[1]
        S = _spec_cols_fwd(xc, nfft, env_f)
        cfg = _SpecCfg(nfft, scale_f, env_f, scale_i, env_i, T, NI, NO, _spec_route(x.dtype, nfft, B, NI, NO))
        if cfg.route == "walk":
            S2, Xs = _spec_mid_walk(S, B, NI, NO, nfft, Hp, False, ctx.needs_input_grad[1], scale_f, 0, 0)
        else:
            S2, Xs = _spec_mid(S, B, NI, NO, nfft, Hp, False, ctx.needs_input_grad[1], True, scale_f, 0, 0)
        key = _grad_cols_key(x, nfft, NI, NO)
        ahead = bool(GRAD_COLS_IN_FORWARD and key in _GRAD_COLS_SEEN and env_i == 0.0 and any(ctx.needs_input_grad[:2]) and
                     _fn("fl_spec_cols_inv_grad_supported", x.dtype)(nfft, NO))
        y, parts, *sg = _spec_cols_inv(S2, B, nfft, nfft, NO, nfft, scale_i, env_i, want_sumsq=True, grad_cols=ahead, sg_buf=S)
        ctx.save_for_backward(Hp, Xs)
        ctx.cfg = cfg
        ctx.speculated = key if ahead else None
        if not y.is_inference():
            y._flamo_sa = _SpectralTag(x, Hrm, Hp, Xs, cfg, parts, y._version, sg[0] if ahead else None)
        return y

    @staticmethod
    def backward(ctx, gy):
        Hp, Xs = ctx.saved_tensors
        if ctx.speculated is not None:
            _GRAD_COLS_SEEN.discard(ctx.speculated)
        return _SpectralApply._backward(ctx.cfg, Hp, Xs, ctx.needs_input_grad[0], ctx.needs_input_grad[1], gy) + (None, None, None, None, None)

    @staticmethod
    def _backward(cfg, Hp, Xkept, need_x, need_h, gy, out_scale=None, host_factor=1.0, Sg=None):
        nfft, NI, NO = cfg.nfft, cfg.NI, cfg.NO
        g = gy.contiguous()
        if g.data_ptr() % (2 * g.element_size()):
            g = g.clone()
        B = g.shape[0]
        kept_sg = Sg is not None
        if Sg is None:
            Sg = _spec_cols_fwd(g, nfft, cfg.env_i, site=1)

        def rows_in():
            return Sg.clone() if kept_sg and need_x else Sg

        route = _spec_backward_route(cfg, _rdtype(Sg), B, need_x, need_h)
        gx = gH = S3 = gYs = None
        if route == "walk":
            if need_h:
                gH = _spec_gradh_walk(Sg, Xkept, B, NI, NO, nfft, cfg.scale_i * host_factor, out_scale)
            if need_x and _walk_applies(nfft, B, NO, NI):
                S3, _ = _spec_mid_walk(Sg, B, NO, NI, nfft, Hp, True, False, cfg.scale_i, 1, 1)
            elif need_x:
                S3, _ = _spec_mid(rows_in(), B, NO, NI, nfft, Hp, True, False, True, cfg.scale_i, 1, 1)
        elif route == "loop":
            gH = _spec_gradh_loop(Sg, Xkept, B, NI, NO, nfft, cfg.scale_i, host_factor, out_scale)
        else:
            S3, gYs = _spec_mid(rows_in(), B, NO, NI if need_x else NO, nfft, Hp if need_x else None, True, need_h, need_x, cfg.scale_i, 1, 1)
        if need_x:
            gx = _spec_cols_inv(S3, B, cfg.T, min(cfg.T, nfft), NI, nfft, cfg.scale_f * host_factor, cfg.env_f, dev_scale=out_scale)
        if gYs is not None:
            gH = _gradh_launch(gYs.movedim(-1, 1), Xkept.movedim(-1, 1), False, host_factor, out_scale).movedim(-1, 0)
        return gx, gH


GRAD_COLS_IN_FORWARD = True
_GRAD_COLS_SEEN = set()


def _grad_cols_key(x, nfft, NI, NO):
    return (int(nfft), int(x.shape[0]), int(NI), int(NO), x.dtype, x.device.index)


class _SpectralMeanSquare(torch.autograd.Function):

    @staticmethod
    def forward(ctx, x, Hrm, y, tag):
        loss = _mean_square_final(tag.parts, y.numel(), y.dtype, y.device)
        ctx.save_for_backward(y, tag.Hp, tag.Xs, tag.Sg)
        ctx.cfg = tag.cfg
        ctx.key = _grad_cols_key(tag.x, tag.cfg.nfft, tag.cfg.NI, tag.cfg.NO)
        return loss

    @staticmethod
    def backward(ctx, gloss):
        y, Hp, Xs, Sg = ctx.saved_tensors
        _GRAD_COLS_SEEN.add(ctx.key)
        c = gloss.to(y.dtype).reshape(())
        gx, gH = _SpectralApply._backward(ctx.cfg, Hp, Xs, ctx.needs_input_grad[0], ctx.needs_input_grad[1], y, c,
                                          2.0 / y.numel(), Sg=Sg)
        return gx, gH, None, None


def spectral_apply(x: torch.Tensor, Hrm: torch.Tensor, nfft: int, norm_f: str = "backward", norm_i: str = "backward",
                   db_f: Optional[float] = None, db_i: Optional[float] = None) -> torch.Tensor:
    if norm_f not in _NORM_FWD or norm_i not in _NORM_INV:
        raise ValueError(f"Invalid normalization mode: {norm_f if norm_f not in _NORM_FWD else norm_i}")
    env_f = 0.0 if not db_f else env_log2_of(db_f, nfft)
    env_i = 0.0 if not db_i else env_log2_of(db_i, nfft)
    return _SpectralApply.apply(x, Hrm, int(nfft), _NORM_FWD[norm_f](nfft), env_f, _NORM_INV[norm_i](nfft), env_i)


def _h_planar(H: torch.Tensor, per_bin: bool) -> torch.Tensor:
    if not per_bin:
        return H
    if _lead_pitch(H.movedim(0, -1)) is not None:
        return H
    M = H.shape[0]
    rest = tuple(H.shape[1:])
    P = _pitch(M)
    out = _transpose(H.contiguous(), 1, M, _prod(rest), P)
    return out.view(*rest, P)[..., :M].movedim(-1, 0)


def _mimo_launch(H, per_bin, diag, conj_t, X):
    real = _rdtype(X)
    B, M, Nx, K, xs_b, xs_n, xs_k = _bnk(X)
    hp = _lead_pitch(H.movedim(0, -1)) if per_bin else 0
    if diag:
        N = H.shape[-1]
        hs_f, hs_n = (1, hp) if per_bin else (0, H.stride(-1))
        Y = _empty_planar(X.shape, X.dtype, X.device)
        _, _, _, _, ys_b, ys_n, ys_k = _bnk(Y)
        fn = _fn("fl_mimo_diag", real, True)
        _lib.check(fn(H.data_ptr(), hs_f, hs_n, int(conj_t), X.data_ptr(), xs_b, xs_n, xs_k, Y.data_ptr(), ys_b, ys_n,
                      ys_k, B, M, N, K, _stream()), "mimo_diag")
        return Y
    No_h, Ni_h = H.shape[-2], H.shape[-1]
    if per_bin:
        hs_f, hs_m, hs_n = 1, Ni_h * hp, hp
    else:
        hs_f, hs_m, hs_n = 0, H.stride(-2), H.stride(-1)
    if conj_t:
        No, Ni, hs_m, hs_n = Ni_h, No_h, hs_n, hs_m
    else:
        No, Ni = No_h, Ni_h
    Y = _empty_planar((B, M, No, *X.shape[3:]), X.dtype, X.device)
    _, _, _, _, ys_b, ys_m, ys_k = _bnk(Y)
    fn = _fn("fl_mimo", real, True)
    tag = ("mimo_bin" if per_bin else "mimo_const") + ("_adj" if conj_t else "_fwd") + f"[cols={B * K},{No}x{Ni}]"
    with kernel_timer.span(tag):
        _lib.check(fn(H.data_ptr(), hs_f, hs_m, hs_n, int(conj_t), X.data_ptr(), xs_b, xs_n, xs_k, Y.data_ptr(), ys_b,
                      ys_m, ys_k, B, M, No, Ni, K, _stream()), "mimo")
    return Y


def _gradh_launch(G, X, diag, scale=1.0, dev_scale=None):
    real = _rdtype(X)
    B, M, Ni, K, xs_b, xs_n, xs_k = _bnk(X)
    _, _, No, _, gs_b, gs_m, gs_k = _bnk(G)
    P = _pitch(M)
    if diag:
        dh = _empty_rows((Ni,), M, X.dtype, X.device)
        fn = _fn("fl_mimo_gradh_diag", real, True)
        _lib.check(fn(G.data_ptr(), gs_b, gs_m, gs_k, X.data_ptr(), xs_b, xs_n, xs_k, dh.data_ptr(), P, B, M, Ni, K,
                      _stream()), "mimo_gradh_diag")
        return dh if scale == 1.0 else dh * scale
    dH = _empty_rows((No, Ni), M, X.dtype, X.device)
    fn = _fn("fl_mimo_gradh", real, True)
    with kernel_timer.span(f"mimo_gradh[cols={B * K},{No}x{Ni}]"):
        if dev_scale is not None:
            if dev_scale.dtype != real or not dev_scale.is_cuda or dev_scale.numel() != 1:
                raise ValueError("mimo_gradh: dev_scale must be one device scalar of the signal's real dtype")
            fn = _fn("fl_mimo_gradh_scaled", real, True)
            _lib.check(fn(G.data_ptr(), gs_b, gs_m, gs_k, X.data_ptr(), xs_b, xs_n, xs_k, dH.data_ptr(), P, float(scale),
                          dev_scale.data_ptr(), B, M, No, Ni, K, _stream()), "mimo_gradh_scaled")
        else:
            _lib.check(fn(G.data_ptr(), gs_b, gs_m, gs_k, X.data_ptr(), xs_b, xs_n, xs_k, dH.data_ptr(), P, float(scale), B, M,
                          No, Ni, K, _stream()), "mimo_gradh")
    return dH


def _gradw_launch(G, X):
# ... 564 lines not shown
    return H, cfg


def _sos_backward_launch(gH, Hf, bc, ac, cfg):
    if cfg.m_local == 0:
        return _zero_part(cfg, bc.device)
    g = _h_planar(gH.resolve_conj(), True)
    g_pitch = _lead_pitch(g.movedim(0, -1))
    L = _lib.lib()
    nblk = L.fl_sos_bwd_blocks(cfg.m_local, cfg.C, cfg.S, int(cfg.real == torch.float32 and Hf is not None))
    part = torch.empty((nblk, 2, 3, cfg.S, cfg.C), dtype=torch.float64, device=bc.device)
    fn = _fn("fl_sos_response_bwd", cfg.real, True)
    Wd = twiddles(cfg.nfft, torch.float64, bc.device)
    with kernel_timer.span("sos_response_bwd"):
        _lib.check(fn(g.data_ptr(), g_pitch, None if Hf is None else Hf.data_ptr(), _pitch(cfg.m_local), bc.data_ptr(),
                      ac.data_ptr(), cfg.S, cfg.C, cfg.gamma, Wd.data_ptr(), cfg.nfft, cfg.bin0, cfg.m_local, part.data_ptr(),
                      _stream()), "sos_response_bwd")
    return part


def _geq_in_kind(t: torch.Tensor, linear: bool, sig: bool = False) -> int:
    if not linear:
        return 0
    return (4 if sig else 2) if t.dtype == torch.float32 else (3 if sig else 1)


def _empty_sections(gains: torch.Tensor):
    b = torch.empty((3, *gains.shape), dtype=torch.float64, device=gains.device)
    return b, torch.empty_like(b)


def _geq_sections_bwd_launch(xc, kind, consts, gb_ptr, ga_ptr, blk_stride, nblk, partW=None, Wr=None):
    nb = xc.shape[0]
    C_ = max(_prod(xc.shape[1:]), 1)
    out = torch.empty_like(xc)
    gW = None if partW is None else torch.empty_like(Wr, memory_format=torch.contiguous_format)
    L = _lib.lib()
    args = (xc.data_ptr(), kind, gb_ptr, ga_ptr, blk_stride, nblk, nb, C_, consts.data_ptr(), out.data_ptr())
    if partW is None:
        _lib.check(L.fl_geq_sections_bwd(*args, _stream()), "geq_sections_bwd")
    else:
        fn = L.fl_geq_sections_bwd_w64 if partW.dtype == torch.float64 else L.fl_geq_sections_bwd_w
        _lib.check(fn(*args, partW.data_ptr(), partW.shape[0] * partW.shape[1], partW.shape[2] * partW.shape[3], gW.data_ptr(),
                      _stream()), "geq_sections_bwd_w")
    return out, gW


class _GeqSections(torch.autograd.Function):
    @staticmethod
    def forward(ctx, gain_db, consts):
        _require_gpu(gain_db, consts)
        gd = gain_db.to(torch.float64).contiguous()
        b, a = _empty_sections(gd)
        _lib.check(_lib.lib().fl_geq_sections(gd.data_ptr(), 0, gd.shape[0], max(_prod(gd.shape[1:]), 1), consts.data_ptr(),
                                              b.data_ptr(), a.data_ptr(), _stream()), "geq_sections")
        ctx.save_for_backward(gd, consts)
        ctx.in_dtype = gain_db.dtype
        return b, a

    @staticmethod
    def backward(ctx, gb, ga):
        gd, consts = ctx.saved_tensors
        gb = torch.zeros_like(gd.new_empty((3, *gd.shape))) if gb is None else gb.to(torch.float64).contiguous()
        ga = torch.zeros_like(gb) if ga is None else ga.to(torch.float64).contiguous()
        out, _ = _geq_sections_bwd_launch(gd, 0, consts, gb.data_ptr(), ga.data_ptr(), 0, 1)
        return out.to(ctx.in_dtype), None


class _Design:
    __slots__ = ()

    def response(self, gamma, nfft, dtype=torch.float32):
        return _Cascade.apply(self, *self.tensors(), float(gamma), int(nfft), dtype)

    def response_rc(self, Wr, gamma, nfft, dtype=torch.float32):
        return _CascadeRC.apply(self, *self.tensors(), Wr.to(dtype), float(gamma), int(nfft), dtype)

    def response_apply(self, X, gamma, nfft, dtype=torch.float32):
        return _CascadeApply.apply(self, *self.tensors(), X, float(gamma), int(nfft), dtype)

    def float_eval(self, ctx):
        return self.float_with_grad or not (ctx.needs_input_grad[1] or ctx.needs_input_grad[2])

    def lanes_grads(self, sec, gH, G, cfg, Wr=None):
        return None


class RawSections(_Design, namedtuple("RawSections", "kind b a")):
    __slots__ = ()
    float_with_grad = False
    n_sections = property(lambda self: self.b.shape[1])
    full = property(lambda self: self.b.dim() == 4)

    def tensors(self):
        return self.b.to(torch.float64), self.a.to(torch.float64)

    def sections(self, b, a, op, prologue):
        if b.shape != a.shape or b.shape[0] != 3 or (b.dim() != 4 if op else b.dim() < 2):
            raise ValueError(f"sos_response{op}: b and a must both be (3, n_sections, {'N_out, N_in' if op else '...'})")
        return (b.contiguous(), a.contiguous()) * 2, None

    def param_grads(self, sec, part, partW=None, Wr=None):
        b, a = sec[2:]
        tot = part.sum(dim=0)
        g = (tot[0].view(b.shape), tot[1].view(a.shape))
        return g if partW is None else g + (partW.sum(dim=(0, 1)).to(Wr.dtype),)


class GeqGains(_Design, namedtuple("GeqGains", "kind x consts gain_map")):
    __slots__ = ()
    float_with_grad = True
    n_sections = property(lambda self: self.x.shape[0])
    full = property(lambda self: self.x.dim() == 3)

    def tensors(self):
        return self.x, self.consts

    def sections(self, x, consts, op, prologue):
        if x.dtype not in (torch.float32, torch.float64):
            raise TypeError(f"geq_cascade{op} expects float32 / float64 parameters")
        xc = x.contiguous()
        if op == "_apply" and xc.dim() != 3:
            raise ValueError(f"geq_cascade{op} expects full (n_bands, N_out, N_in) parameters")
        b, a = _empty_sections(xc)
        geq = (xc, _geq_in_kind(xc, True, _is_sigmoid(self.gain_map)), consts)
        if not prologue:
            _lib.check(_lib.lib().fl_geq_sections(xc.data_ptr(), geq[1], xc.shape[0], max(_prod(xc.shape[1:]), 1),
                                                  consts.data_ptr(), b.data_ptr(), a.data_ptr(), _stream()), "geq_sections")
        return (xc, consts, b, a), geq if prologue else None

    def lanes_grads(self, sec, gH, G, cfg, Wr=None):
        if G is None:
            return None
        mode = int(Wr is not None)
        No, Nmid, Ni = (G.shape[0], G.shape[1], Wr.shape[1]) if mode else (cfg.C, 1, 0)
        nbx = _geq_lanes_blocks(cfg, Nmid, Ni, mode)
        if nbx <= 0:
            return None
        xc, consts, b, a = sec
        out, gW = _geq_backward_lanes(mode, gH, G, b, a, Wr, cfg, No, Nmid, Ni, nbx, xc, consts, _is_sigmoid(self.gain_map))
        return (out, None, gW) if mode else (out, None)

    def param_grads(self, sec, part, partW=None, Wr=None):
        xc, consts = sec[:2]
        st = part.shape[3] * part.shape[4]
        out, gW = _geq_sections_bwd_launch(xc, _geq_in_kind(xc, True, _is_sigmoid(self.gain_map)), consts, part.data_ptr(),
                                           part.data_ptr() + 3 * st * part.element_size(), 6 * st, part.shape[0], partW, Wr)
        return (out, None) if partW is None else (out, None, gW)


class _Cascade(torch.autograd.Function):

    @staticmethod
    def forward(ctx, design, p, q, gamma, nfft, real):
        _require_gpu(p, q)
        ctx.design = design
        sec, geq = design.sections(p, q, "", prologue=real == torch.float32)
        H, ctx.cfg = _sos_forward_launch(*sec[2:], gamma, nfft, real, design.float_eval(ctx), geq)
        keep = [H] if (real == torch.float64 or SOS_BWD_MIXED) else []
        ctx.save_for_backward(*sec, *keep)
        return H.movedim(-1, 0)

    @staticmethod
    def backward(ctx, gH):
        sec, kept = ctx.saved_tensors[:4], ctx.saved_tensors[4:]
        Hf = kept[0] if kept else None
        g = ctx.design.lanes_grads(sec, gH, Hf, ctx.cfg)
        if g is None:
            g = ctx.design.param_grads(sec, _sos_backward_launch(gH, Hf, *sec[2:], ctx.cfg))
        return (None, *g, None, None, None)


def cascade_apply_supported(real: torch.dtype, X: torch.Tensor) -> bool:
    return real == torch.float32 and SOS_BWD_MIXED and X.dim() == 3 and X.dtype == torch.complex64 and X.is_cuda


def _sos_apply_forward(bc, ac, Xp, gamma, nfft, real, float_eval):
    S, No, Ni = bc.shape[1], bc.shape[2], bc.shape[3]
    B = Xp.shape[0]
    L = _lib.lib()
    cfg = _cascade_cfg(gamma, nfft, S, No * Ni, real)
    m_local = cfg.m_local
    if m_local == 0 or not (float_eval and FLOAT_CASCADE_EVAL and real == torch.float32 and B <= 2
                            and Ni <= L.fl_sos_response_apply_max_ni(S)):
        H, cfg = _sos_forward_launch(bc, ac, gamma, nfft, real, float_eval)
        if m_local == 0:
            return H, _empty_planar((B, 0, No), _cdtype(real), bc.device), cfg
        return H, _mimo_launch(H.movedim(-1, 0), True, False, False, Xp), cfg
    dev = bc.device
    _, M, Nx, K, xs_b, xs_n, _ = _bnk(Xp)
    assert K == 1 and Nx == Ni and M == m_local
    H = _empty_rows((No, Ni), m_local, torch.complex64, dev)
    Y = _empty_planar((B, m_local, No), torch.complex64, dev)
    _, _, _, _, ys_b, ys_m, _ = _bnk(Y)
    with kernel_timer.span("sos_response"):
        _lib.check(L.fl_sos_response_apply_c64(bc.data_ptr(), ac.data_ptr(), S, No, Ni, Xp.data_ptr(), xs_b, xs_n, B, cfg.gamma,
                                               twiddles(nfft, torch.float64, dev).data_ptr(), nfft, cfg.bin0, m_local, H.data_ptr(),
                                               _pitch(m_local), Y.data_ptr(), ys_b, ys_m, _stream()), "sos_response_apply")
    return H, Y, cfg


def _sos_backward_outer_launch(gY, Xp, Hf, bc, ac, cfg, No, Ni):
    if cfg.m_local == 0:
        return _zero_part(cfg, bc.device)
    B, M, _, K, xs_b, xs_n, _ = _bnk(Xp)
    _, _, _, _, gs_b, gs_n, _ = _bnk(gY)
    assert K == 1 and cfg.C == No * Ni and M == cfg.m_local
    L = _lib.lib()
    part = torch.empty((L.fl_sos_bwd_blocks(cfg.m_local, cfg.C, cfg.S, 1), 2, 3, cfg.S, cfg.C), dtype=torch.float64, device=bc.device)
    with kernel_timer.span("sos_response_bwd"):
        _lib.check(L.fl_sos_response_bwd_outer_c64(gY.data_ptr(), gs_b, gs_n, Xp.data_ptr(), xs_b, xs_n, B, No, Ni, Hf.data_ptr(),
                                                   _pitch(cfg.m_local), bc.data_ptr(), ac.data_ptr(), cfg.S, cfg.gamma,
                                                   twiddles(cfg.nfft, torch.float64, bc.device).data_ptr(), cfg.nfft, cfg.bin0,
                                                   cfg.m_local, part.data_ptr(), _stream()), "sos_response_bwd_outer")
    return part


class _CascadeApply(torch.autograd.Function):

    @staticmethod
    def forward(ctx, design, p, q, X, gamma, nfft, real):
        _require_gpu(p, q, X)
        ctx.design = design
# ... 26 lines not shown

def cascade_rc_supported(real: torch.dtype, n_in: int, n_mid: int = 1, n_sections: int = 1) -> bool:
    if int(n_in) not in (2, 4, 8, 16):
        return False
    n_mid, n_sections = int(n_mid), int(n_sections)
    if n_mid < 1 or n_mid > 32 or n_sections < 1 or n_sections > 64:
        return False
    if real == torch.float64:
        return n_sections <= 12 and n_mid * 6 * n_sections * 8 + n_mid * int(n_in) * 8 <= 64 * 1024
    if not (real == torch.float32 and SOS_BWD_MIXED):
        return False
    return n_mid * 6 * n_sections * 8 + n_mid * int(n_in) * 4 <= 64 * 1024


def _cascade_rc_forward(b, a, Wr, gamma, nfft, real, float_eval, geq=None):
    if b.dim() != 4:
        raise ValueError("cascade_rc expects a full (N_out, N_mid) cascade")
    dev = b.device
    S, No, Nmid = b.shape[1], b.shape[2], b.shape[3]
    if Wr.dim() != 2 or Wr.shape[0] != Nmid:
        raise ValueError(f"cascade_rc: the constant factor must be ({Nmid}, N_in), got {tuple(Wr.shape)}")
    Ni = Wr.shape[1]
    cfg = _cascade_cfg(gamma, nfft, S, No * Nmid, real)
    f64 = real == torch.float64
    G = _empty_rows((No, Nmid), cfg.m_local, _cdtype(real), dev)
    H = _empty_rows((No, Ni), cfg.m_local, _cdtype(real), dev)
    Wc = Wr.contiguous()
    Wd = twiddles(nfft, torch.float64, dev)
    P = _pitch(cfg.m_local)
    if cfg.m_local == 0 and geq is None:
        return H.movedim(-1, 0), G, cfg
    with kernel_timer.span("sos_response_rc"):
        if geq is not None:
            xc, kind, consts = geq
            fn, name = _fn("fl_geq_response_rc", real, True), "geq_response_rc"
            args = (xc.data_ptr(), kind, S, consts.data_ptr(), b.data_ptr(), a.data_ptr())
        else:
            fn, name = _fn("fl_sos_response_rc", real, True), "sos_response_rc"
            args = (b.data_ptr(), a.data_ptr(), S)
        args += (No, Nmid, Ni, Wc.data_ptr(), cfg.gamma, Wd.data_ptr(), nfft, cfg.bin0, cfg.m_local, G.data_ptr(), P, H.data_ptr(), P)
        if not f64:
            args += (int(bool(float_eval and FLOAT_CASCADE_EVAL)),)
        _lib.check(fn(*args, _stream()), name)
    if getattr(_lib._pair, "stream_of", None) is not None and _lib.lib(pair_ok=True).fl_launch_pair_pending():
        _pair_keep((b, a, Wc, Wd, G, H) + ((geq[0], geq[2]) if geq is not None else ()))
        if kernel_timer.enabled:
            kernel_timer.drop_last("sos_response_rc")
    return H.movedim(-1, 0), G, cfg


def _cascade_rc_backward(gH, G, b, a, Wr, cfg):
    real = cfg.real
    No, Nmid = G.shape[0], G.shape[1]
    Ni = Wr.shape[1]
    if cfg.m_local == 0:
        return _zero_part(cfg, b.device), torch.zeros((1, No, Nmid, Ni), dtype=real, device=b.device)
    g = _h_planar(gH.resolve_conj(), True)
    L = _lib.lib()
    nblk = L.fl_sos_bwd_blocks(cfg.m_local, cfg.C, cfg.S, 0 if real == torch.float64 else 1)
    part = torch.empty((nblk, 2, 3, cfg.S, cfg.C), dtype=torch.float64, device=b.device)
    partW = torch.empty((nblk, No, Nmid, Ni), dtype=real, device=b.device)
    Wc = Wr.contiguous()
    fn = _fn("fl_sos_response_bwd_rc", real, True)
    with kernel_timer.span("sos_response_bwd_rc"):
        _lib.check(fn(g.data_ptr(), _lead_pitch(g.movedim(0, -1)), G.data_ptr(), _pitch(cfg.m_local),
                      b.data_ptr(), a.data_ptr(), cfg.S, No, Nmid, Ni, Wc.data_ptr(), cfg.gamma,
                      twiddles(cfg.nfft, torch.float64, b.device).data_ptr(), cfg.nfft, cfg.bin0, cfg.m_local,
                      part.data_ptr(), partW.data_ptr(), _stream()), "sos_response_bwd_rc")
    return part, partW


LANES_F64_ROW_MAJOR_RC = False


def _geq_lanes_blocks(cfg, ppr: int, niw: int, mode: int) -> int:
    if not SOS_BWD_MIXED:
        return 0
    if cfg.real == torch.float64 and mode == 1 and cfg.bin0 < 0 and not LANES_F64_ROW_MAJOR_RC:
        return 0
    fn = _lib.lib().fl_geq_bwd_lanes_blocks if cfg.real == torch.float32 else _lib.lib().fl_geq_bwd_lanes_blocks_f64
    return int(fn(cfg.m_local, cfg.C, cfg.S, cfg.nfft, cfg.bin0, int(ppr), int(niw), int(mode)))


def _geq_backward_lanes(mode, gH, G, b, a, Wr, cfg, No, Nmid, Ni, nbx, xc, consts, sig):
    gamma, nfft, S, C_, bin0, m_local, real = cfg
    dev = b.device
    g = _h_planar(gH.resolve_conj(), True)
    L = _lib.lib()
    f64 = real == torch.float64
    psum = torch.empty((S * C_, nbx, 4), dtype=real, device=dev)
    pq = torch.empty((C_, nbx), dtype=real, device=dev)
    wrows = (L.fl_geq_bwd_lanes_wrows_f64 if f64 else L.fl_geq_bwd_lanes_wrows)(m_local, C_, S, nfft, bin0, Nmid, Ni) if mode == 1 else 0
    partW = torch.empty((Nmid * Ni, wrows), dtype=real, device=dev) if mode == 1 else None
    Wc = Wr.to(real).contiguous() if mode == 1 else None
    with kernel_timer.span("sos_response_bwd_rc" if mode == 1 else "sos_response_bwd"):
        _lib.check(_fn("fl_geq_response_bwd_lanes", real, True)(
            mode, g.data_ptr(), _lead_pitch(g.movedim(0, -1)), G.data_ptr(), _pitch(m_local), b.data_ptr(), a.data_ptr(), S, No, Nmid, Ni,
            None if Wc is None else Wc.data_ptr(), gamma, twiddles(nfft, torch.float64, dev).data_ptr(), nfft, bin0, m_local,
            psum.data_ptr(), pq.data_ptr(), None if partW is None else partW.data_ptr(), _stream()), "geq_response_bwd_lanes")
    out = torch.empty_like(xc)
    gW = torch.empty(Wr.shape, dtype=real, device=dev) if mode == 1 else None
    _lib.check((L.fl_geq_sections_bwd_lanes_f64 if f64 else L.fl_geq_sections_bwd_lanes)(
        xc.data_ptr(), _geq_in_kind(xc, True, sig), psum.data_ptr(), pq.data_ptr(), nbx, b.data_ptr(), a.data_ptr(), gamma, S, C_,
        consts.data_ptr(), out.data_ptr(), None if partW is None else partW.data_ptr(), wrows, Nmid * Ni if mode == 1 else 0,
        None if gW is None else gW.data_ptr(), _stream()), "geq_sections_bwd_lanes")
    if gW is not None and gW.dtype != Wr.dtype:
        gW = gW.to(Wr.dtype)
    return out, gW


class _CascadeRC(torch.autograd.Function):

    @staticmethod
    def forward(ctx, design, p, q, Wr, gamma, nfft, real):
        _require_gpu(p, q, Wr)
        ctx.design = design
        sec, geq = design.sections(p, q, "_rc", prologue=True)
        H, G, ctx.cfg = _cascade_rc_forward(*sec[2:], Wr, gamma, nfft, real, design.float_eval(ctx), geq=geq)
        ctx.save_for_backward(*sec, G, Wr)
        return H

    @staticmethod
    def backward(ctx, gH):
        *sec, G, Wr = ctx.saved_tensors
        g = ctx.design.lanes_grads(sec, gH, G, ctx.cfg, Wr)
        if g is None:
            g = ctx.design.param_grads(sec, *_cascade_rc_backward(gH, G, *sec[2:], Wr, ctx.cfg), Wr)
        return (None, *g, None, None, None)


def sos_response_rc(b, a, Wr, gamma: float, nfft: int, dtype=torch.float32) -> torch.Tensor:
    return RawSections("sos", b, a).response_rc(Wr, gamma, nfft, dtype)


def geq_cascade_rc(x, consts, Wr, gamma: float, nfft: int, dtype=torch.float32, gain_map: str = "abs") -> torch.Tensor:
    return GeqGains("geq", x, consts, gain_map).response_rc(Wr, gamma, nfft, dtype)


def _is_sigmoid(gain_map: str) -> bool:
    if gain_map not in ("abs", "sigmoid"):
        raise ValueError("gain_map: 'abs' (20 log10|x|, the module default) or 'sigmoid' (20 log10(sigmoid(x)))")
    return gain_map == "sigmoid"


def geq_cascade(x: torch.Tensor, consts: torch.Tensor, gamma: float, nfft: int, dtype=torch.float32, gain_map: str = "abs") -> torch.Tensor:
    return GeqGains("geq", x, consts, gain_map).response(gamma, nfft, dtype)


def geq_sections(gain_db: torch.Tensor, consts: torch.Tensor):
    return _GeqSections.apply(gain_db, consts)


def sos_response(b: torch.Tensor, a: torch.Tensor, gamma: float, nfft: int, dtype=torch.float32) -> torch.Tensor:
    return RawSections("sos", b, a).response(gamma, nfft, dtype)


_ms_scratch = {}


def _ms_scratch_for(dev: torch.device) -> torch.Tensor:
    key = (dev.index, torch.cuda.current_stream(dev).cuda_stream)
    s = _ms_scratch.get(key)
    if s is None:
        s = torch.empty(_lib.lib().fl_mean_square_scratch_bytes(), dtype=torch.uint8, device=dev)
        _ms_scratch[key] = s
    return s


def _rows_of(y: torch.Tensor):
    if y.is_contiguous():
        return y, 1, y.numel(), y.numel()
    if y.dim() >= 2:
        mem = y.movedim(1, -1)
        P = _lead_pitch(mem)
        if P is not None:
            return y, _prod(mem.shape[:-1]), mem.shape[-1], P
    yc = y.contiguous()
    return yc, 1, yc.numel(), yc.numel()


class _MeanSquare(torch.autograd.Function):
    @staticmethod
    def forward(ctx, y):
        dev = _require_gpu(y)
        if y.dtype not in (torch.float32, torch.float64):
            raise TypeError("mean_square expects a real float32/float64 tensor")
        if y.numel() == 0:
            raise ValueError("mean_square of an empty tensor")
        ym, rows, cols, pitch = _rows_of(y)
        loss = torch.empty((), dtype=y.dtype, device=dev)
        fn = _fn("fl_mean_square", y.dtype)
        with kernel_timer.span("mean_square"):
            _lib.check(fn(ym.data_ptr(), rows, cols, pitch, loss.data_ptr(), _ms_scratch_for(dev).data_ptr(), _stream()),
                       "mean_square")
        ctx.save_for_backward(ym)
        ctx.layout = (rows, cols, pitch)
        return loss

    @staticmethod
    def backward(ctx, gloss):
        (ym,) = ctx.saved_tensors
        rows, cols, pitch = ctx.layout
        gy = torch.empty_strided(ym.shape, ym.stride(), dtype=ym.dtype, device=ym.device)
        g = gloss.to(ym.dtype).contiguous()
        fn = _fn("fl_mean_square_bwd", ym.dtype)
        with kernel_timer.span("mean_square_bwd"):
            _lib.check(fn(ym.data_ptr(), g.data_ptr(), gy.data_ptr(), rows, cols, pitch, _stream()), "mean_square_bwd")
        return gy


def _mean_square_final(parts, n, real, dev):
# ... 291 lines not shown
```

include/flamo_hip.h:

```cpp
#ifndef FLAMO_HIP_H
#define FLAMO_HIP_H

#include <stddef.h>
#include <stdint.h>

#ifdef __cplusplus
extern "C" {
#endif

#define FL_OK 0
#define FL_ERR_BAD_ARG (-1)
#define FL_ERR_UNSUPPORTED (-2)
#define FL_ERR_HIP (-3)

#define FL_ABI_VERSION 1

int fl_version(void);
const char* fl_last_error(void);


int fl_twiddle_fill_f32(void* W, int nfft, void* stream);
int fl_twiddle_fill_f64(void* W, int nfft, void* stream);

int fl_fft_plan(int nfft, int is_f64, int* L1, int* L2);
size_t fl_fft_scratch_elems(int nfft, int is_f64, int nsig);
int fl_debug_set_fft_max_single(int max_half_len);
int fl_debug_set_fft_fast(int enabled);

int fl_rfft_f32(const void* x, long x_sig_stride, int t_in, void* X, long X_sig_stride, void* scratch, const void* W,
                int nsig, int nfft, double scale, double env_log2, int interior_x2, void* stream);
int fl_rfft_f64(const void* x, long x_sig_stride, int t_in, void* X, long X_sig_stride, void* scratch, const void* W,
                int nsig, int nfft, double scale, double env_log2, int interior_x2, void* stream);

int fl_rfft_ci_f32(const void* x, int n_chan, int t_in, void* X, long X_sig_stride, void* scratch, const void* W,
                   int nsig, int nfft, double scale, double env_log2, int interior_x2, void* stream);
int fl_rfft_ci_f64(const void* x, int n_chan, int t_in, void* X, long X_sig_stride, void* scratch, const void* W,
                   int nsig, int nfft, double scale, double env_log2, int interior_x2, void* stream);

int fl_irfft_f32(const void* X, long X_sig_stride, void* y, long y_sig_stride, int t_out, void* scratch, const void* W,
                 int nsig, int nfft, double scale, double env_log2, int interior_half, void* stream);
int fl_irfft_f64(const void* X, long X_sig_stride, void* y, long y_sig_stride, int t_out, void* scratch, const void* W,
                 int nsig, int nfft, double scale, double env_log2, int interior_half, void* stream);

int fl_transpose(const void* src, void* dst, int nbatch, int rows, int cols, long dst_pitch, int elem_bytes, void* stream);

int fl_spec_plan(int nfft, int* L1, int* L2);
size_t fl_spec_aux_elems(int nfft);
int fl_spec_aux_fill_f32(void* W, int nfft, void* stream);
int fl_spec_supports(int nfft, int n_in, int n_out);
int fl_debug_set_spec(int vt, int rg);
int fl_debug_set_spec_times(void* buf);
int fl_spec_cols_fwd_f32(const void* x, int Bn, int t_len, int G, void* S, const void* W, int nfft, double env_log2,
                         void* stream);
int fl_spec_mid_f32(const void* S, void* S2, void* Xs, long xs_b, long xs_n, const void* H, long hs_m, long hs_n, int conj_h,
                    const void* W, int nfft, int Bn, int NI, int NO, double spec_scale, int spec_interior2, int pre_half,
                    void* stream);
int fl_spec_walk_supports(int nfft, int n_in, int n_out);
size_t fl_spec_walk_spectrum_elems(int nfft, int Bn, int NI);
int fl_spec_walk_workgroups(int nfft, int Bn);
int fl_spec_walk_partition(int nfft, int Bn, int n_wg, int* bounds);
int fl_spec_mid_walk_f32(const void* S, void* S2, void* Xp, const void* H, long hs_m, long hs_n, int conj_h, const void* W, int nfft, int Bn,
                         int NI, int NO, double spec_scale, int spec_interior2, int pre_half, const void* bounds, void* stream);
int fl_spec_gradh_slices(int nfft, int Bn);
int fl_spec_gradh_walk_f32(const void* Sg, const void* Xp, void* dH_parts, long ds_s, long ds_m, long ds_n, int n_slices, const void* W,
                           int nfft, int Bn, int NI, int NO, double scale_g, int interior2_g, const void* out_scale, void* stream);
int fl_sum_parts_c64(const void* parts, long part_stride, int n_parts, void* out, long n, void* stream);
int fl_debug_set_walk(int mode, int wgs, int slices, void* times);
int fl_debug_set_walk_stamps(void* buf);
int fl_wall_clock_khz(void);
int fl_spec_cols_inv_f32(const void* S2, void* y, int Bn, int t_len, int t_out, int G, const void* W, int nfft, double scale,
                         double env_log2, void* sumsq_parts, const void* dev_scale, void* Sg, void* stream);
int fl_spec_cols_blocks_f32(int nfft, int Bn, int G);
int fl_spec_cols_inv_grad_supported_f32(int nfft, int G);
int fl_spec_cols_inv_inplace_ok_f32(int nfft, int G);
int fl_permute_bins_c64(const void* src, long src_pitch, void* dst, long dst_pitch, int nplanes, int nfft, int inverse,
                        void* stream);
int fl_spec_gradh_loop_supports_f32(int nfft, int NI, int NO);
int fl_spec_gradh_loop_supports_f64(int nfft, int NI, int NO);
int fl_spec_gradh_loop_f32(const void* Sg, const void* Xs, long xs_b, long xs_n, void* dH, long ds_m, long ds_n, const void* W,
                           int nfft, int Bn, int NI, int NO, double scale_g, int interior2, double out_scale,
                           const void* dev_scale, void* stream);
int fl_spec_gradh_loop_f64(const void* Sg, const void* Xs, long xs_b, long xs_n, void* dH, long ds_m, long ds_n, const void* W,
                           int nfft, int Bn, int NI, int NO, double scale_g, int interior2, double out_scale,
                           const void* dev_scale, void* stream);

int fl_spec_supports_f64(int nfft, int n_in, int n_out);
int fl_spec_aux_fill_f64(void* W, int nfft, void* stream);
int fl_spec_cols_fwd_f64(const void* x, int Bn, int t_len, int G, void* S, const void* W, int nfft, double env_log2,
                         void* stream);
int fl_spec_mid_f64(const void* S, void* S2, void* Xs, long xs_b, long xs_n, const void* H, long hs_m, long hs_n, int conj_h,
                    const void* W, int nfft, int Bn, int NI, int NO, double spec_scale, int spec_interior2, int pre_half,
                    void* stream);
int fl_spec_cols_inv_f64(const void* S2, void* y, int Bn, int t_len, int t_out, int G, const void* W, int nfft, double scale,
                         double env_log2, void* sumsq_parts, const void* dev_scale, void* Sg, void* stream);
int fl_spec_cols_blocks_f64(int nfft, int Bn, int G);
int fl_spec_cols_inv_grad_supported_f64(int nfft, int G);
int fl_spec_cols_inv_inplace_ok_f64(int nfft, int G);
int fl_permute_bins_c128(const void* src, long src_pitch, void* dst, long dst_pitch, int nplanes, int nfft, int inverse,
                         void* stream);

int fl_mimo_c64(const void* H, long hs_f, long hs_m, long hs_n, int conj_h,
                const void* X, long xs_b, long xs_n, long xs_k,
                void* Y, long ys_b, long ys_m, long ys_k,
                int B, int M, int No, int Ni, int K, void* stream);
int fl_mimo_c128(const void* H, long hs_f, long hs_m, long hs_n, int conj_h,
                 const void* X, long xs_b, long xs_n, long xs_k,
                 void* Y, long ys_b, long ys_m, long ys_k,
                 int B, int M, int No, int Ni, int K, void* stream);

int fl_mimo_diag_c64(const void* h, long hs_f, long hs_n, int conj_h,
                     const void* X, long xs_b, long xs_n, long xs_k,
                     void* Y, long ys_b, long ys_n, long ys_k,
                     int B, int M, int N, int K, void* stream);
int fl_mimo_diag_c128(const void* h, long hs_f, long hs_n, int conj_h,
                      const void* X, long xs_b, long xs_n, long xs_k,
                      void* Y, long ys_b, long ys_n, long ys_k,
                      int B, int M, int N, int K, void* stream);

int fl_mimo_gradh_c64(const void* G, long gs_b, long gs_m, long gs_k,
                      const void* X, long xs_b, long xs_n, long xs_k,
                      void* dH, long dh_pitch, double scale, int B, int M, int No, int Ni, int K, void* stream);
int fl_mimo_gradh_c128(const void* G, long gs_b, long gs_m, long gs_k,
                       const void* X, long xs_b, long xs_n, long xs_k,
                       void* dH, long dh_pitch, double scale, int B, int M, int No, int Ni, int K, void* stream);
int fl_mimo_gradh_scaled_c64(const void* G, long gs_b, long gs_m, long gs_k, const void* X, long xs_b, long xs_n, long xs_k,
                             void* dH, long dh_pitch, double scale, const void* dev_scale, int B, int M, int No, int Ni, int K, void* stream);
int fl_mimo_gradh_scaled_c128(const void* G, long gs_b, long gs_m, long gs_k, const void* X, long xs_b, long xs_n, long xs_k,
                              void* dH, long dh_pitch, double scale, const void* dev_scale, int B, int M, int No, int Ni, int K, void* stream);
int fl_mimo_gradh_diag_c64(const void* G, long gs_b, long gs_n, long gs_k,
                           const void* X, long xs_b, long xs_n, long xs_k,
                           void* dh, long dh_pitch, int B, int M, int N, int K, void* stream);
int fl_mimo_gradh_diag_c128(const void* G, long gs_b, long gs_n, long gs_k,
                            const void* X, long xs_b, long xs_n, long xs_k,
                            void* dh, long dh_pitch, int B, int M, int N, int K, void* stream);

int fl_mimo_gradw_blocks(int M);
int fl_debug_set_mimo_variant(int variant, int gradw_cap);
int fl_mimo_gradw_c64(const void* G, long gs_b, long gs_m, long gs_k, const void* X, long xs_b, long xs_n, long xs_k,
                      void* part, void* dW, int B, int M, int No, int Ni, int K, void* stream);
int fl_mimo_gradw_c128(const void* G, long gs_b, long gs_m, long gs_k, const void* X, long xs_b, long xs_n, long xs_k,
                       void* part, void* dW, int B, int M, int No, int Ni, int K, void* stream);
int fl_mimo_gradw_re_c64(const void* G, long gs_b, long gs_m, long gs_k, const void* X, long xs_b, long xs_n, long xs_k,
                         void* part, void* dW, int B, int M, int No, int Ni, int K, void* stream);
int fl_mimo_gradw_re_c128(const void* G, long gs_b, long gs_m, long gs_k, const void* X, long xs_b, long xs_n, long xs_k,
                          void* part, void* dW, int B, int M, int No, int Ni, int K, void* stream);

int fl_delay_response_c64(const int32_t* m, const void* amp, int C, const void* W, int nfft,
                          int bin0, int m_local, void* H, long h_pitch, void* stream);
int fl_delay_response_c128(const int32_t* m, const void* amp, int C, const void* W, int nfft,
                           int bin0, int m_local, void* H, long h_pitch, void* stream);

int fl_sos_response_c64(const void* b, const void* a, int S, int C, double gamma, const void* Wd,
                        int nfft, int bin0, int m_local, void* H, long h_pitch, void* stream);
int fl_sos_response_c128(const void* b, const void* a, int S, int C, double gamma, const void* Wd,
                         int nfft, int bin0, int m_local, void* H, long h_pitch, void* stream);
int fl_sos_response_f32eval_c64(const void* b, const void* a, int S, int C, double gamma, const void* Wd,
                                int nfft, int bin0, int m_local, void* H, long h_pitch, void* stream);
int fl_geq_response_c64(const void* gain, int in_kind, int nb, const void* consts, void* b, void* a, int C, double gamma, const void* Wd,
                        int nfft, int bin0, int m_local, void* H, long h_pitch, int float_eval, void* stream);
int fl_sos_bwd_blocks(int m_local, int C, int S, int mixed);
int fl_debug_set_sos_chunk(int sections_per_thread);
int fl_debug_set_rc_fast(int on);
int fl_sos_response_bwd_c64(const void* gH, long g_pitch, const void* H, long h_pitch, const void* b, const void* a, int S,
                            int C, double gamma, const void* Wd, int nfft, int bin0, int m_local, void* part, void* stream);
int fl_sos_response_bwd_c128(const void* gH, long g_pitch, const void* H, long h_pitch, const void* b, const void* a, int S,
                             int C, double gamma, const void* Wd, int nfft, int bin0, int m_local, void* part, void* stream);
int fl_sos_response_apply_max_ni(int S);
int fl_sos_response_apply_c64(const void* b, const void* a, int S, int No, int Ni, const void* X, long xs_b, long xs_n, int BX,
                              double gamma, const void* Wd, int nfft, int bin0, int m_local, void* G, long g_pitch, void* Y, long ys_b,
                              long ys_m, void* stream);
int fl_sos_response_bwd_outer_c64(const void* gY, long gy_sb, long gy_sn, const void* X, long x_sb, long x_sn, int B, int No, int Ni,
                                  const void* H, long h_pitch, const void* b, const void* a, int S, double gamma, const void* Wd,
                                  int nfft, int bin0, int m_local, void* part, void* stream);
int fl_sos_response_rc_c64(const void* b, const void* a, int S, int No, int Nmid, int Ni, const void* Wr, double gamma,
                           const void* Wd, int nfft, int bin0, int m_local, void* G, long g_pitch, void* H, long h_pitch,
                           int float_eval, void* stream);
int fl_geq_response_rc_c64(const void* gain, int in_kind, int nb, const void* consts, void* b, void* a, int No, int Nmid, int Ni,
                           const void* Wr, double gamma, const void* Wd, int nfft, int bin0, int m_local, void* G, long g_pitch,
                           void* H, long h_pitch, int float_eval, void* stream);
int fl_sos_response_bwd_rc_c64(const void* gHfull, long g_pitch, const void* G, long h_pitch, const void* b, const void* a,
                               int S, int No, int Nmid, int Ni, const void* Wr, double gamma, const void* Wd, int nfft,
                               int bin0, int m_local, void* part, void* partW, void* stream);
int fl_sos_response_rc_c128(const void* b, const void* a, int S, int No, int Nmid, int Ni, const void* Wr, double gamma,
                            const void* Wd, int nfft, int bin0, int m_local, void* G, long g_pitch, void* H, long h_pitch,
                            void* stream);
int fl_geq_response_rc_c128(const void* gain, int in_kind, int nb, const void* consts, void* b, void* a, int No, int Nmid, int Ni,
                            const void* Wr, double gamma, const void* Wd, int nfft, int bin0, int m_local, void* G, long g_pitch,
                            void* H, long h_pitch, void* stream);
int fl_sos_response_bwd_rc_c128(const void* gHfull, long g_pitch, const void* G, long h_pitch, const void* b, const void* a,
                                int S, int No, int Nmid, int Ni, const void* Wr, double gamma, const void* Wd, int nfft,
                                int bin0, int m_local, void* part, void* partW, void* stream);

int fl_geq_sections(const void* gain, int in_kind, int nb, int C, const void* consts, void* b, void* a, void* stream);
int fl_geq_sections_bwd(const void* gain, int in_kind, const void* gb, const void* ga, long blk_stride, int nblk, int nb,
                        int C, const void* consts, void* ggain, void* stream);
int fl_geq_sections_bwd_w(const void* gain, int in_kind, const void* gb, const void* ga, long blk_stride, int nblk, int nb,
                          int C, const void* consts, void* ggain, const void* partW, int wrows, int wn, void* gW, void* stream);
int fl_geq_sections_bwd_w64(const void* gain, int in_kind, const void* gb, const void* ga, long blk_stride, int nblk, int nb,
                            int C, const void* consts, void* ggain, const void* partW, int wrows, int wn, void* gW, void* stream);

int fl_geq_bwd_lanes_blocks(int m_local, int C, int S, int nfft, int bin0, int ppr, int niw, int mode);
int fl_geq_bwd_lanes_wrows(int m_local, int C, int S, int nfft, int bin0, int ppr, int niw);
int fl_geq_response_bwd_lanes_c64(int mode, const void* gH, long g_pitch, const void* G, long h_pitch, const void* b, const void* a,
                                  int S, int No, int Nmid, int Ni, const void* Wr, double gamma, const void* Wd, int nfft,
                                  int bin0, int m_local, void* psum, void* pq, void* partW, void* stream);
int fl_geq_sections_bwd_lanes(const void* gain, int in_kind, const void* psum, const void* pq, int nbx, const void* b, const void* a,
                              double gamma, int nb, int C, const void* consts, void* ggain, const void* partW, int wrows, int wn,
                              void* gW, void* stream);
int fl_geq_bwd_lanes_blocks_f64(int m_local, int C, int S, int nfft, int bin0, int ppr, int niw, int mode);
int fl_geq_bwd_lanes_wrows_f64(int m_local, int C, int S, int nfft, int bin0, int ppr, int niw);
int fl_geq_response_bwd_lanes_c128(int mode, const void* gH, long g_pitch, const void* G, long h_pitch, const void* b, const void* a,
                                   int S, int No, int Nmid, int Ni, const void* Wr, double gamma, const void* Wd, int nfft,
                                   int bin0, int m_local, void* psum, void* pq, void* partW, void* stream);
int fl_geq_sections_bwd_lanes_f64(const void* gain, int in_kind, const void* psum, const void* pq, int nbx, const void* b, const void* a,
                                  double gamma, int nb, int C, const void* consts, void* ggain, const void* partW, int wrows, int wn,
                                  void* gW, void* stream);
int fl_debug_set_cascade_lanes(int on, int blocks_per_cu, int tile_bins);
int fl_debug_set_cascade_stamps(void* device_buffer, int skip);

int fl_solve_max_n(int f64);
int fl_solve_c64(const void* P, long p_pitch, int one_minus, int adjoint,
                 const void* R, long rs_b, long rs_n, long rs_k,
                 void* OUT, long os_b, long os_n, long os_k,
                 int B, int M, int N, int K, void* stream);
int fl_solve_c128(const void* P, long p_pitch, int one_minus, int adjoint,
                  const void* R, long rs_b, long rs_n, long rs_k,
                  void* OUT, long os_b, long os_n, long os_k,
                  int B, int M, int N, int K, void* stream);

int fl_solve_ws_max_n(void);
long fl_solve_ws_bytes(int N, int M, int f64);
int fl_solve_ws_c64(const void* P, long p_pitch, int one_minus, int adjoint,
                    const void* R, long rs_b, long rs_n, long rs_k,
                    void* OUT, long os_b, long os_n, long os_k,
                    int B, int M, int N, int K, void* ws, long ws_bytes, void* stream);
int fl_solve_ws_c128(const void* P, long p_pitch, int one_minus, int adjoint,
                     const void* R, long rs_b, long rs_n, long rs_k,
                     void* OUT, long os_b, long os_n, long os_k,
                     int B, int M, int N, int K, void* ws, long ws_bytes, void* stream);

int fl_solve_scaled_c64(const void* P, long p_pitch, const void* l, long l_sn, int adjoint, const void* R, long rs_b, long rs_n,
                        long rs_k, void* OUT, long os_b, long os_n, long os_k, int B, int M, int N, int K, void* stream);
int fl_solve_scaled_c128(const void* P, long p_pitch, const void* l, long l_sn, int adjoint, const void* R, long rs_b, long rs_n,
                         long rs_k, void* OUT, long os_b, long os_n, long os_k, int B, int M, int N, int K, void* stream);

size_t fl_solve_kept_lu_elems(int N, int M, int f64);
size_t fl_solve_kept_piv_elems(int N, int M, int f64);
int fl_solve_scaled_keep_c64(const void* P, long p_pitch, const void* l, long l_sn, const void* R, long rs_b, long rs_n, long rs_k, void* OUT,
                             long os_b, long os_n, long os_k, int B, int M, int N, int K, void* LU, void* piv, void* stream);
int fl_solve_scaled_keep_c128(const void* P, long p_pitch, const void* l, long l_sn, const void* R, long rs_b, long rs_n, long rs_k, void* OUT,
                              long os_b, long os_n, long os_k, int B, int M, int N, int K, void* LU, void* piv, void* stream);
int fl_solve_kept_adjoint_c64(const void* LU, const void* piv, const void* R, long rs_b, long rs_n, long rs_k,
                              void* OUT, long os_b, long os_n, long os_k, int B, int M, int N, int K, void* stream);
int fl_solve_kept_adjoint_c128(const void* LU, const void* piv, const void* R, long rs_b, long rs_n, long rs_k,
                               void* OUT, long os_b, long os_n, long os_k, int B, int M, int N, int K, void* stream);
int fl_solve_fdn_keep_tile(int N, int f64);
int fl_solve_fdn_wadj_supported(int N);
int fl_solve_dud2_grads_w_c64(const void* l, long l_sn, long l_sf, const void* l2, long l2_sn, long l2_sf, const void* U, const void* r,
                              long r_sn, long r_sf, const void* W, long w_sn, const void* gy, long gy_sb, const void* OUT, long s_b,
                              long s_n, long s_k, int B, int M, int N, void* gl, long gl_sn, void* gr, long gr_sn, void* partU,
                              void* gU, void* gR0, const void* sx, long sx_b, const void* sy, long sy_b, void* g_side_real,
                              void* stream);
int fl_solve_dud2_grads_w_c128(const void* l, long l_sn, long l_sf, const void* l2, long l2_sn, long l2_sf, const void* U, const void* r,
                              long r_sn, long r_sf, const void* W, long w_sn, const void* gy, long gy_sb, const void* OUT, long s_b,
                              long s_n, long s_k, int B, int M, int N, void* gl, long gl_sn, void* gr, long gr_sn, void* partU,
                              void* gU, void* gR0, const void* sx, long sx_b, const void* sy, long sy_b, void* g_side_real,
                              void* stream);
int fl_solve_fdn_wadj_c64(const void* l, long l_sn, long l_sf, const void* l2, long l2_sn, long l2_sf, const void* U, const void* r,
                          long r_sn, long r_sf, const void* rv, int rv_real, const void* rs, long rs_sb, const void* cw, int cw_real,
                          void* cz, long cz_sb, void* OUT, long os_b, long os_n, long os_k, int B, int M, int N, void* wadj, long wadj_sn,
                          void* stream);
int fl_solve_fdn_wadj_c128(const void* l, long l_sn, long l_sf, const void* l2, long l2_sn, long l2_sf, const void* U, const void* r,
                          long r_sn, long r_sf, const void* rv, int rv_real, const void* rs, long rs_sb, const void* cw, int cw_real,
                          void* cz, long cz_sb, void* OUT, long os_b, long os_n, long os_k, int B, int M, int N, void* wadj, long wadj_sn,
                          void* stream);
int fl_solve_fdn_keep_c64(const void* l, long l_sn, long l_sf, const void* l2, long l2_sn, long l2_sf, const void* U, const void* r,
                          long r_sn, long r_sf, const void* rv, int rv_real, const void* rs, long rs_sb, const void* cw, int cw_real,
                          void* cz, long cz_sb, void* OUT, long os_b, long os_n, long os_k, int B, int M, int N, void* LU, void* piv,
                          void* stream);
int fl_solve_fdn_keep_c128(const void* l, long l_sn, long l_sf, const void* l2, long l2_sn, long l2_sf, const void* U, const void* r,
                           long r_sn, long r_sf, const void* rv, int rv_real, const void* rs, long rs_sb, const void* cw, int cw_real,
                           void* cz, long cz_sb, void* OUT, long os_b, long os_n, long os_k, int B, int M, int N, void* LU, void* piv,
                           void* stream);
int fl_solve_kept_adjoint_rank1_c64(const void* LU, const void* piv, int tile_bins, const void* rv, int rv_real, const void* rs, long rs_sb,
                                    void* OUT, long os_b, long os_n, long os_k, int B, int M, int N, void* stream);
int fl_solve_kept_adjoint_rank1_c128(const void* LU, const void* piv, int tile_bins, const void* rv, int rv_real, const void* rs, long rs_sb,
                                     void* OUT, long os_b, long os_n, long os_k, int B, int M, int N, void* stream);

// ... 91 lines not shown
```

Measured before the change: 681.2 billion products/s.

## Balance gradh walk with piece table and fuse partial-plane sum into GEQ backward

Adds a per-block piece table for the spectral gradient walk kernel so batch slices can be split unevenly across planes. A host-side greedy load-balance model over CUs picks the split. The GEQ lanes backward kernel gains a multi-plane variant that reads the 2 or 3 partial cotangent planes directly and sums them in registers. This removes the separate sum_parts reduction and its extra memory pass. In exchange it adds a host planning step, memoization, and handoff logic in Python that matches tensors by pointer.

```diff
diff --git a/flamo_amd/_lib.py b/flamo_amd/_lib.py
--- a/flamo_amd/_lib.py
+++ b/flamo_amd/_lib.py
@@ -54,6 +54,9 @@
     "fl_spec_gradh_slices": (_i, [_i, _i]),
     "fl_spec_gradh_walk_f32": (_i, [_vp, _vp, _vp, _l, _l, _l, _i, _vp, _i, _i, _i, _i, _d, _i, _vp, _vp]),
     "fl_sum_parts_c64": (_i, [_vp, _l, _i, _vp, _l, _vp]),
+    "fl_spec_gradh_pieces": (_i, [_i, _i, _i, _i, C.POINTER(_i), C.POINTER(_i)]),
+    "fl_spec_gradh_walk_pieces_f32": (_i, [_vp, _vp, _vp, _l, _l, _l, _vp, _i, _i, _i, _vp, _i, _i, _i, _i, _d, _i, _vp, _vp]),
+    "fl_debug_set_gradh_pieces": (_i, [_i, _i, _i]),
     "fl_debug_set_walk": (_i, [_i, _i, _i, _vp]),
     "fl_debug_set_walk_stamps": (_i, [_vp]),
     "fl_wall_clock_khz": (_i, []),
@@ -113,6 +116,7 @@
     "fl_geq_bwd_lanes_blocks": (_i, [_i, _i, _i, _i, _i, _i, _i, _i]),
     "fl_geq_bwd_lanes_wrows": (_i, [_i, _i, _i, _i, _i, _i, _i]),
     "fl_geq_response_bwd_lanes_c64": (_i, [_i, _vp, _l, _vp, _l, _vp, _vp, _i, _i, _i, _i, _vp, _d, _vp, _i, _i, _i, _vp, _vp, _vp, _vp]),
+    "fl_geq_response_bwd_lanes_planes_c64": (_i, [_i, _vp, _l, _i, _l, _vp, _l, _vp, _vp, _i, _i, _i, _i, _vp, _d, _vp, _i, _i, _i, _vp, _vp, _vp, _vp]),
     "fl_geq_sections_bwd_lanes": (_i, [_vp, _i, _vp, _vp, _i, _vp, _vp, _d, _i, _i, _vp, _vp, _vp, _i, _i, _vp, _vp]),
     "fl_geq_bwd_lanes_blocks_f64": (_i, [_i, _i, _i, _i, _i, _i, _i, _i]),
     "fl_geq_bwd_lanes_wrows_f64": (_i, [_i, _i, _i, _i, _i, _i, _i]),
diff --git a/flamo_amd/csrc/cascade2.hip b/flamo_amd/csrc/cascade2.hip
--- a/flamo_amd/csrc/cascade2.hip
+++ b/flamo_amd/csrc/cascade2.hip
@@ -42,6 +42,7 @@
     long long* stamps;
     int skip;
     unsigned pol;
+    long g_plane;
 };
 
 template <int NSUM, typename P2, typename T>
@@ -64,7 +65,7 @@
     }
 }
 
-template <typename RT, int NIW, int PPR, int NSUM, bool OUTER>
+template <typename RT, int NIW, int PPR, int NSUM, bool OUTER, int NPL = 1>
 __global__ void __launch_bounds__(sizeof(RT) == 8 ? 384 : 768, sizeof(RT) == 8 ? 2 : 3) sos_bwd_lanes_kernel(const LanesArgs<RT> A) {
     typedef typename Vec<RT>::v2 P2;
     typedef typename Vec<RT>::v4 P4;
@@ -142,6 +143,7 @@
     constexpr int TRIPS = (RC || OUTER) ? 1 : 4;
     struct Item {
         cT gv[NG];
+        cT gx[NPL > 1 ? (NPL - 1) * NG : 1];
         cT hv[JPT];
         cx<double> w1;
     };
@@ -201,6 +203,19 @@
 #pragma unroll
                     for (int nn = 0; nn < NG; ++nn) pre[q].gv[nn] = at(A.gH + (size_t)nn * A.g_pitch, goff);
                 }
+                if constexpr (NPL > 1) {
+#pragma unroll
+                    for (int pl = 1; pl < NPL; ++pl) {
+                        const cT* gp = A.gH + (size_t)pl * A.g_plane;
+                        if (A.pol & POL_LANES_GH_NT) {
+#pragma unroll
+                            for (int nn = 0; nn < NG; ++nn) pre[q].gx[(pl - 1) * NG + nn] = at_nt(gp + (size_t)nn * A.g_pitch, goff);
+                        } else {
+#pragma unroll
+                            for (int nn = 0; nn < NG; ++nn) pre[q].gx[(pl - 1) * NG + nn] = at(gp + (size_t)nn * A.g_pitch, goff);
+                        }
+                    }
+                }
                 if (A.pol & POL_LANES_G_NT) {
 #pragma unroll
                     for (int j = 0; j < JPT; ++j) pre[q].hv[j] = at_nt(A.G + (size_t)j * A.h_pitch, hoff);
@@ -233,6 +248,15 @@
                 if constexpr (NSUM == 3) B.us[i] = (RT)(1.0 - P.w1.x);
             }
             if constexpr (RC) {
+                if constexpr (NPL > 1) {
+#pragma unroll
+                    for (int nn = 0; nn < NG; ++nn)
+#pragma unroll
+                        for (int pl = 1; pl < NPL; ++pl) {
+                            pre[q].gv[nn].x += pre[q].gx[(pl - 1) * NG + nn].x;
+                            pre[q].gv[nn].y += pre[q].gx[(pl - 1) * NG + nn].y;
+                        }
+                }
 #pragma unroll
                 for (int j = 0; j < JPT; ++j) {
                     P2 gi = {(RT)0.0, (RT)0.0};
@@ -680,11 +704,14 @@
     const LanesPlan P = lanes_plan(m_local, C, S, nfft, bin0, ppr, niw, 1);
     return P.ok ? P.nbx * P.ng : 0;
 }
-FL_ENTRY_C64_C128(fl_geq_response_bwd_lanes, (int mode, const void* gH, long g_pitch, const void* G, long h_pitch, const void* b, const void* a,
-                                              int S, int No, int Nmid, int Ni, const void* Wr, double gamma, const void* Wd, int nfft,
-                                              int bin0, int m_local, void* psum, void* pq, void* partW, void* stream),
-                  (mode, gH, g_pitch, G, h_pitch, b, a, S, No, Nmid, Ni, Wr, gamma, Wd, nfft, bin0, m_local, psum, pq, partW, stream)) {
+template <typename T>
+static int lanes_response_bwd_impl(int mode, const void* gH, long g_pitch, const void* G, long h_pitch, const void* b, const void* a, int S,
+                                   int No, int Nmid, int Ni, const void* Wr, double gamma, const void* Wd, int nfft, int bin0, int m_local,
+                                   void* psum, void* pq, void* partW, void* stream, int n_planes, long g_plane) {
     FL_REQUIRE(mode == 0 || mode == 1, "geq_response_bwd_lanes: mode 0 (plain) or 1 (constant factor)");
+    FL_REQUIRE(n_planes == 1 || (sizeof(T) == 4 && mode == 1 && (n_planes == 2 || n_planes == 3) && Ni <= 8 &&
+                                 g_plane >= (long)No * Ni * g_pitch && (size_t)n_planes * (size_t)g_plane * 8 < (1ull << 40)),
+               "geq_response_bwd_lanes: 2 or 3 cotangent plane sets, float32 constant-factor mode with 2 / 4 / 8 columns only");
     FL_REQUIRE(gH && G && b && a && Wd && psum && pq, "geq_response_bwd_lanes: null pointer");
     FL_REQUIRE(mode == 0 || (Wr && partW), "geq_response_bwd_lanes: the constant-factor mode needs Wr and partW");
     FL_REQUIRE(g_pitch >= m_local && h_pitch >= m_local, "geq_response_bwd_lanes: pitches must be >= m_local");
@@ -698,7 +725,7 @@
     A.b = (const double*)b; A.a = (const double*)a; A.S = S; A.C = C; A.g = gamma; A.Wd = (const cx<double>*)Wd;
     A.nfft = nfft; A.bin0 = bin0; A.m_local = m_local; A.gH = (const cx<T>*)gH; A.g_pitch = g_pitch;
     A.G = (const cx<T>*)G; A.h_pitch = h_pitch; A.Wr = (const T*)Wr; A.psum = (T*)psum; A.pq = (T*)pq;
-    A.partW = (T*)partW;
+    A.partW = (T*)partW; A.g_plane = g_plane;
     A.stamps = g_lanes_stamps;
     A.skip = g_lanes_skip;
     A.pol = stream_policy();
@@ -710,6 +737,16 @@
         constexpr int niw = decltype(NIW)::value;
         static bool done[kMaxDevices] = {};
         auto kern = sos_bwd_lanes_kernel<T, niw, niw ? niw : 1, 2, false>;
+        if constexpr (sizeof(T) == 4 && (niw == 2 || niw == 4 || niw == 8)) {
+            if (n_planes > 1) {
+                static bool done_p[2][kMaxDevices] = {};
+                const LanesArgs<float>& Af = reinterpret_cast<const LanesArgs<float>&>(A);
+                auto kp = n_planes == 2 ? sos_bwd_lanes_kernel<float, niw, niw, 2, false, 2> : sos_bwd_lanes_kernel<float, niw, niw, 2, false, 3>;
+                rc = lanes_ensure_lds(reinterpret_cast<const void*>(kp), lds, done_p[n_planes - 2]);
+                if (rc == FL_OK) hipLaunchKernelGGL(kp, grid, block, lds, (hipStream_t)stream, Af);
+                return;
+            }
+        }
         rc = lanes_ensure_lds(reinterpret_cast<const void*>(kern), lds, done);
         if (rc == FL_OK) hipLaunchKernelGGL(kern, grid, block, lds, (hipStream_t)stream, A);
     });
@@ -717,6 +754,20 @@
     FL_CHECK_LAUNCH("geq_response_bwd_lanes");
     return FL_OK;
 }
+FL_ENTRY_C64_C128(fl_geq_response_bwd_lanes, (int mode, const void* gH, long g_pitch, const void* G, long h_pitch, const void* b, const void* a,
+                                              int S, int No, int Nmid, int Ni, const void* Wr, double gamma, const void* Wd, int nfft,
+                                              int bin0, int m_local, void* psum, void* pq, void* partW, void* stream),
+                  (mode, gH, g_pitch, G, h_pitch, b, a, S, No, Nmid, Ni, Wr, gamma, Wd, nfft, bin0, m_local, psum, pq, partW, stream)) {
+    return lanes_response_bwd_impl<T>(mode, gH, g_pitch, G, h_pitch, b, a, S, No, Nmid, Ni, Wr, gamma, Wd, nfft, bin0, m_local, psum, pq,
+                                      partW, stream, 1, 0);
+}
+extern "C" int fl_geq_response_bwd_lanes_planes_c64(int mode, const void* gH, long g_pitch, int n_planes, long g_plane, const void* G,
+                                                    long h_pitch, const void* b, const void* a, int S, int No, int Nmid, int Ni,
+                                                    const void* Wr, double gamma, const void* Wd, int nfft, int bin0, int m_local,
+                                                    void* psum, void* pq, void* partW, void* stream) {
+    return lanes_response_bwd_impl<float>(mode, gH, g_pitch, G, h_pitch, b, a, S, No, Nmid, Ni, Wr, gamma, Wd, nfft, bin0, m_local, psum,
+                                          pq, partW, stream, n_planes, g_plane);
+}
 extern "C" int fl_geq_sections_bwd_lanes(const void* gain, int in_kind, const void* psum, const void* pq, int nbx, const void* b, const void* a,
                                          double gamma, int nb, int C, const void* consts, void* ggain, const void* partW, int wrows, int wn,
                                          void* gW, void* stream) {
diff --git a/flamo_amd/csrc/specwalk.hip b/flamo_amd/csrc/specwalk.hip
--- a/flamo_amd/csrc/specwalk.hip
+++ b/flamo_amd/csrc/specwalk.hip
@@ -1,4 +1,8 @@
 #include "spectral_common.h"
+#include <algorithm>
+#include <cstring>
+#include <mutex>
+#include <vector>
 
 namespace fl {
 using namespace sp32;
@@ -426,6 +430,9 @@
 #undef FL_STAMP
 }
 
+struct GradhPiece {
+    int r, cg, b_lo, n_it, plane, pad[3];
+};
 struct GradhArgs {
     const cf* Sg;
     const cf* Xp;
@@ -438,6 +445,7 @@
     int interior2_g;
     long long* dbg_times;
     unsigned pol;
+    const GradhPiece* pieces;
 };
 
 template <int A, int B, int NI, int NO, int NSC, int OCC, int DEPTH, bool DBG = false>
@@ -468,11 +476,15 @@
     const int grp = wave >> 2;
     const int P = a.L1 / 2 + 1;
     const int xcd = blockIdx.x & 7, q_ = blockIdx.x >> 3;
-    const int r = (q_ / (a.NS * NSC)) * 8 + xcd, sl = (q_ / NSC) % a.NS, mo = (q_ % NSC) * NOL;
+    int r = (q_ / (a.NS * NSC)) * 8 + xcd, sl = (q_ / NSC) % a.NS, mo = (q_ % NSC) * NOL;
+    int b_lo = (int)((long)a.Bn * sl / a.NS), n_it = (int)((long)a.Bn * (sl + 1) / a.NS) - b_lo;
+    if (a.pieces) {
+        const GradhPiece pc = a.pieces[blockIdx.x];
+        r = pc.r, sl = pc.plane, mo = pc.cg * NOL, b_lo = pc.b_lo, n_it = pc.n_it;
+    }
     if (r >= P) return;
     const int rm = (a.L1 - r) % a.L1;
     const bool selfm = rm == r;
-    const int b_lo = (int)((long)a.Bn * sl / a.NS), n_it = (int)((long)a.Bn * (sl + 1) / a.NS) - b_lo;
     const size_t bstride_g = (size_t)a.L1 * a.L2 * NO;
     const unsigned sg_lds = lds_addr_of(stage_g), sx_lds = lds_addr_of(stage_x);
 
@@ -711,6 +723,7 @@
 static int g_walk_slices = 0;
 static long long* g_walk_times = nullptr;
 static long long* g_walk_stamps = nullptr;
+static int g_gradh_force[3] = {0, 0, 0};
 static int g_walk_nsc = 2;
 static int g_walk_fc = [] { const char* e = getenv("FLAMO_WALK_FC"); return e ? atoi(e) : 38; }();
 static int g_walk_fc2 = [] { const char* e = getenv("FLAMO_WALK_FC2"); return e ? atoi(e) : 38; }();
@@ -801,8 +814,15 @@
     return ns < Bn ? ns : Bn;
 }
 
-int fl_spec_gradh_walk_f32(const void* Sg, const void* Xp, void* dH_parts, long ds_s, long ds_m, long ds_n, int n_slices, const void* W,
-                           int nfft, int Bn, int NI, int NO, double scale_g, int interior2_g, const void* out_scale, void* stream) {
+static int gradh_nsc(int l2, int NI, int NO) {
+    if (NO == 2) return 1;
+    if (NI == 8 && NO == 8 && l2 == 240 && g_walk_nsc != 2) return g_walk_nsc;
+    return 2;
+}
+
+static int gradh_launch(const void* Sg, const void* Xp, void* dH_parts, long ds_s, long ds_m, long ds_n, int n_slices, const void* pieces,
+                        int n_records, int nsc, const void* W, int nfft, int Bn, int NI, int NO, double scale_g, int interior2_g,
+                        const void* out_scale, void* stream) {
     FL_REQUIRE(Sg && Xp && dH_parts && W, "spec_gradh_walk: null pointer");
     FL_REQUIRE(n_slices >= 1 && n_slices <= (Bn > 0 ? Bn : 1), "spec_gradh_walk: slices must be in [1, batch]");
     FL_REQUIRE(reinterpret_cast<uintptr_t>(Sg) % 16 == 0 && reinterpret_cast<uintptr_t>(Xp) % 16 == 0, "spec_gradh_walk: scratch arrays must be 16-byte aligned");
@@ -814,7 +834,9 @@
     a.W = (const cf*)W; a.n = nfft; a.L = nfft / 2; a.Bn = Bn; a.NS = n_slices;
     a.scale_g = (float)scale_g; a.interior2_g = interior2_g; a.dbg_times = g_walk_times; a.out_scale = (const float*)out_scale;
     a.pol = stream_policy();
+    a.pieces = (const GradhPiece*)pieces;
     FL_REQUIRE((size_t)NO * (size_t)ds_m * 8ull < (1ull << 32), "spec_gradh_walk: a partial plane set exceeds 32-bit offsets");
+    FL_REQUIRE(!pieces || (n_records > 0 && nsc == gradh_nsc(a.L2, NI, NO)), "spec_gradh_walk: the piece table was built for another kernel form");
     const int P = a.L1 / 2 + 1;
     hipStream_t st = (hipStream_t)stream;
     int lrc = FL_ERR_UNSUPPORTED;
@@ -824,7 +846,7 @@
         constexpr size_t lds = ((size_t)3 * 2 * NOL * LENP + DEPTH_ * (((2 * B_ * NOL + 63) / 64) * A_ * 64 + 8 * NI_ * 64) +    \
                                 ((B_ * tw_pitch(A_) + 1) & ~1) + LEN) * sizeof(cf);                                              \
         static_assert(lds <= 160 * 1024, "LDS budget");                                                                          \
-        const unsigned nblk = (unsigned)(cdiv_i(P, 8) * 8 * n_slices * NSC_);                                                    \
+        const unsigned nblk = pieces ? (unsigned)n_records : (unsigned)(cdiv_i(P, 8) * 8 * n_slices * NSC_);                     \
         auto kern = spec_gradh_walk<A_, B_, NI_, NO_, NSC_, OCC_, DEPTH_>;                                                       \
         auto kern_dbg = spec_gradh_walk<A_, B_, NI_, NO_, NSC_, OCC_, DEPTH_, true>;                                             \
         static bool done[kMaxDevices] = {}, done_dbg[kMaxDevices] = {};                                                          \
@@ -861,6 +883,87 @@
     if (lrc) return lrc;
     FL_CHECK_LAUNCH("spec_gradh_walk");
     return FL_OK;
+}
+
+int fl_spec_gradh_walk_f32(const void* Sg, const void* Xp, void* dH_parts, long ds_s, long ds_m, long ds_n, int n_slices, const void* W,
+                           int nfft, int Bn, int NI, int NO, double scale_g, int interior2_g, const void* out_scale, void* stream) {
+    return gradh_launch(Sg, Xp, dH_parts, ds_s, ds_m, ds_n, n_slices, nullptr, 0, 0, W, nfft, Bn, NI, NO, scale_g, interior2_g, out_scale, stream);
+}
+
+int fl_spec_gradh_walk_pieces_f32(const void* Sg, const void* Xp, void* dH_parts, long ds_s, long ds_m, long ds_n, const void* pieces,
+                                  int n_records, int n_planes, int nsc, const void* W, int nfft, int Bn, int NI, int NO, double scale_g,
+                                  int interior2_g, const void* out_scale, void* stream) {
+    FL_REQUIRE(pieces && reinterpret_cast<uintptr_t>(pieces) % 16 == 0, "spec_gradh_walk_pieces: no piece table");
+    return gradh_launch(Sg, Xp, dH_parts, ds_s, ds_m, ds_n, n_planes, pieces, n_records, nsc, W, nfft, Bn, NI, NO, scale_g, interior2_g, out_scale, stream);
+}
+
+int fl_debug_set_gradh_pieces(int n0, int n1, int n2) {
+    g_gradh_force[0] = n0; g_gradh_force[1] = n1; g_gradh_force[2] = n2;
+    return FL_OK;
+}
+
+int fl_spec_gradh_pieces(int nfft, int Bn, int NI, int NO, int* records, int* info) {
+    int L1, L2;
+    if (!info || spec_plan(nfft, L1, L2) != FL_OK || Bn <= 0 || !g_walk || !walk_shape(L2, NI, NO)) return 0;
+    const int nsc = gradh_nsc(L2, NI, NO);
+    if (nsc != 1 && nsc != 2) return 0;
+    const int P = L1 / 2 + 1, cus = device_cus() / 8 > 0 ? device_cus() / 8 : 1;
+    const bool forced = g_gradh_force[0] > 0;
+    const int np = forced ? (g_gradh_force[2] > 0 ? 3 : g_gradh_force[1] > 0 ? 2 : 1) : (nsc == 1 ? 3 : 2);
+    if (Bn < np) return 0;
+    auto ends = [&](const int* sz, int n_sz) {
+        long worst = 0;
+        std::vector<long> cu(cus);
+        for (int x = 0; x < 8 && x < P; ++x) {
+            std::fill(cu.begin(), cu.end(), 0L);
+            for (int j = 0; j < n_sz; ++j)
+                for (int r = x; r < P; r += 8)
+                    for (int c = 0; c < nsc; ++c) {
+                        auto it = std::min_element(cu.begin(), cu.end());
+                        *it += (long)(sz[j] + 2) * ((r == 0 || 2 * r == L1) ? g_walk_us : 20);
+                    }
+            worst = std::max(worst, *std::max_element(cu.begin(), cu.end()));
+        }
+        return worst;
+    };
+    int best[3] = {0, 0, 0};
+    if (forced) {
+        int tot = 0;
+        for (int j = 0; j < np; ++j) best[j] = g_gradh_force[j], tot += best[j];
+        if (tot != Bn) return 0;
+    } else {
+        static int memo_key[7] = {0, 0, 0, 0, 0, 0, 0}, memo[3] = {0, 0, 0};
+        static std::mutex memo_mx;
+        const int key[7] = {nfft, Bn, NI, NO, nsc, cus, g_walk_us};
+        std::lock_guard<std::mutex> lock(memo_mx);
+        if (std::memcmp(key, memo_key, sizeof key)) {
+            const int whole = Bn;
+            long t_best = ends(&whole, 1) * 9 / 10 + 1;
+            memo[0] = memo[1] = memo[2] = 0;
+            for (int n0 = 1; n0 <= Bn - np + 1; ++n0)
+                for (int n1 = np == 3 ? 1 : Bn - n0; n1 <= n0 && n0 + n1 <= Bn - (np - 2); ++n1) {
+                    const int sz[3] = {n0, n1, Bn - n0 - n1};
+                    if ((np == 3 && (sz[2] < 1 || sz[2] > n1)) || (np == 2 && n1 < 1)) continue;
+                    const long t = ends(sz, np);
+                    if (t < t_best) t_best = t, memo[0] = sz[0], memo[1] = sz[1], memo[2] = sz[2];
+                }
+            std::memcpy(memo_key, key, sizeof key);
+        }
+        if (!memo[0]) return 0;
+        for (int j = 0; j < 3; ++j) best[j] = memo[j];
+    }
+    info[0] = np; info[1] = nsc; info[2] = best[0]; info[3] = best[1]; info[4] = best[2];
+    const int per_xcd = cdiv_i(P, 8) * nsc * np, n_rec = 8 * per_xcd;
+    if (records) {
+        GradhPiece* rec = reinterpret_cast<GradhPiece*>(records);
+        for (int x = 0; x < 8; ++x) {
+            int i = 0;
+            for (int j = 0, b_lo = 0; j < np; b_lo += best[j], ++j)
+                for (int r = x; r < cdiv_i(P, 8) * 8; r += 8)
+                    for (int c = 0; c < nsc; ++c) rec[8 * i++ + x] = GradhPiece{r < P ? r : P, c, b_lo, best[j], j, {0, 0, 0}};
+        }
+    }
+    return n_rec;
 }
 
 int fl_sum_parts_c64(const void* parts, long part_stride, int n_parts, void* out, long n, void* stream) {
diff --git a/flamo_amd/ops.py b/flamo_amd/ops.py
--- a/flamo_amd/ops.py
+++ b/flamo_amd/ops.py
@@ -865,11 +865,71 @@
     return dH.movedim(-1, 0)
 
 
-def _spec_gradh_walk(Sg, Xp, B, NI, NO, nfft, scale_g, out_scale=None):
+_gradh_tables = {}
+
+
+def _gradh_pieces(nfft: int, B: int, NI: int, NO: int, dev: torch.device):
+    L = _lib.lib()
+    info = (ctypes.c_int * 5)()
+    n_rec = int(L.fl_spec_gradh_pieces(nfft, B, NI, NO, None, info))
+    if n_rec <= 0:
+        return None
+    key = (int(nfft), int(B), int(NI), int(NO), n_rec, tuple(info), dev.index if dev.index is not None else torch.cuda.current_device())
+    t = _gradh_tables.get(key)
+    if t is None:
+        if torch.cuda.is_current_stream_capturing():
+            return None
+        host = (ctypes.c_int * (8 * n_rec))()
+        if int(L.fl_spec_gradh_pieces(nfft, B, NI, NO, host, info)) != n_rec:
+            raise RuntimeError("spec_gradh_pieces: the table changed between the count and the fill")
+        t = torch.tensor(list(host), dtype=torch.int32).to(dev)
+        torch.cuda.current_stream(dev).synchronize()
+        _gradh_tables[key] = t
+    return t, n_rec, int(info[0]), int(info[1])
+
+
+GRADH_PIECES = True
+
+
+def _gradh_consumer(Hrm, cfg, B, need_x, need_h):
+    if not (GRADH_PIECES and cfg.route == "walk" and need_h and not need_x):
+        return None
+    node = Hrm.grad_fn
+    if node is None or not isinstance(node, _CascadeRC._backward_cls) or Hrm._backward_hooks or Hrm.retains_grad:
+        return None
+    if node.cfg.real != torch.float32 or Hrm.dtype != torch.complex64:
+        return None
+    *_, G, Wr = node.saved_tensors
+    if not node.design.lanes_blocks(G, node.cfg, Wr) or Wr.shape[1] not in (2, 4, 8):
+        return None
+    if tuple(Hrm.shape[1:]) != (G.shape[0], Wr.shape[1]) or _gradh_pieces(cfg.nfft, B, cfg.NI, cfg.NO, Hrm.device) is None:
+        return None
+    return node
+
+
+def _graph_task():
+    return torch._C._current_graph_task_id()
+
+
+def _spec_gradh_walk(Sg, Xp, B, NI, NO, nfft, scale_g, out_scale=None, consumer=None):
     dev = Sg.device
     L = _lib.lib()
     M = nfft // 2 + 1
     P = _pitch(M)
+    pieces = None
+    if consumer is not None and GRADH_PIECES and _graph_task() >= 0:
+        pieces = _gradh_pieces(nfft, B, NI, NO, dev)
+    if pieces is not None:
+        table, n_rec, npl, nsc = pieces
+        parts = torch.empty((npl, NO, NI, P), dtype=torch.complex64, device=dev)
+        with kernel_timer.span("spec_gradh_walk"):
+            _lib.check(L.fl_spec_gradh_walk_pieces_f32(Sg.data_ptr(), Xp.data_ptr(), parts.data_ptr(), NO * NI * P, NI * P, P,
+                                                       table.data_ptr(), n_rec, npl, nsc, twiddles(nfft, torch.float32, dev).data_ptr(),
+                                                       nfft, B, NI, NO, scale_g, 1, _ptr(out_scale), _stream()), "spec_gradh_walk")
+        pending = consumer.__dict__.setdefault("_gh_parts", [])
+        pending[:] = [e for e in pending if e[0] == _graph_task()]
+        pending.append((_graph_task(), parts, M))
+        return parts[0][..., :M].movedim(-1, 0)
     ns = int(L.fl_spec_gradh_slices(nfft, B))
     parts = torch.empty((ns, NO, NI, P), dtype=torch.complex64, device=dev)
     with kernel_timer.span("spec_gradh_walk"):
@@ -909,7 +969,7 @@
     return "layered"
 
 
-_SpectralTag = namedtuple("_SpectralTag", "x Hrm Hp Xs cfg parts version Sg")
+_SpectralTag = namedtuple("_SpectralTag", "x Hrm Hp Xs cfg parts version Sg consumer", defaults=(None,))
 
 
 class _SpectralApply(torch.autograd.Function):
@@ -941,9 +1001,10 @@
         y, parts, *sg = _spec_cols_inv(S2, B, nfft, nfft, NO, nfft, scale_i, env_i, want_sumsq=True, grad_cols=ahead, sg_buf=S)
         ctx.save_for_backward(Hp, Xs)
         ctx.cfg = cfg
+        ctx.consumer = _gradh_consumer(Hrm, cfg, B, ctx.needs_input_grad[0], ctx.needs_input_grad[1]) if Xs is not None else None
         ctx.speculated = key if ahead else None
         if not y.is_inference():
-            y._flamo_sa = _SpectralTag(x, Hrm, Hp, Xs, cfg, parts, y._version, sg[0] if ahead else None)
+            y._flamo_sa = _SpectralTag(x, Hrm, Hp, Xs, cfg, parts, y._version, sg[0] if ahead else None, ctx.consumer)
         return y
 
     @staticmethod
@@ -951,10 +1012,11 @@
         Hp, Xs = ctx.saved_tensors
         if ctx.speculated is not None:
             _GRAD_COLS_SEEN.discard(ctx.speculated)
-        return _SpectralApply._backward(ctx.cfg, Hp, Xs, ctx.needs_input_grad[0], ctx.needs_input_grad[1], gy) + (None, None, None, None, None)
-
-    @staticmethod
-    def _backward(cfg, Hp, Xkept, need_x, need_h, gy, out_scale=None, host_factor=1.0, Sg=None):
+        return _SpectralApply._backward(ctx.cfg, Hp, Xs, ctx.needs_input_grad[0], ctx.needs_input_grad[1], gy,
+                                        consumer=ctx.consumer) + (None, None, None, None, None)
+
+    @staticmethod
+    def _backward(cfg, Hp, Xkept, need_x, need_h, gy, out_scale=None, host_factor=1.0, Sg=None, consumer=None):
         nfft, NI, NO = cfg.nfft, cfg.NI, cfg.NO
         g = gy.contiguous()
         if g.data_ptr() % (2 * g.element_size()):
@@ -971,7 +1033,8 @@
         gx = gH = S3 = gYs = None
         if route == "walk":
             if need_h:
-                gH = _spec_gradh_walk(Sg, Xkept, B, NI, NO, nfft, cfg.scale_i * host_factor, out_scale)
+                gH = _spec_gradh_walk(Sg, Xkept, B, NI, NO, nfft, cfg.scale_i * host_factor, out_scale,
+                                      consumer=None if need_x else consumer)
             if need_x and _walk_applies(nfft, B, NO, NI):
                 S3, _ = _spec_mid_walk(Sg, B, NO, NI, nfft, Hp, True, False, cfg.scale_i, 1, 1)
             elif need_x:
@@ -1003,6 +1066,7 @@
         ctx.save_for_backward(y, tag.Hp, tag.Xs, tag.Sg)
         ctx.cfg = tag.cfg
         ctx.key = _grad_cols_key(tag.x, tag.cfg.nfft, tag.cfg.NI, tag.cfg.NO)
+        ctx.consumer = tag.consumer if tag.Hrm is Hrm else None
         return loss
 
     @staticmethod
@@ -1011,7 +1075,7 @@
         _GRAD_COLS_SEEN.add(ctx.key)
         c = gloss.to(y.dtype).reshape(())
         gx, gH = _SpectralApply._backward(ctx.cfg, Hp, Xs, ctx.needs_input_grad[0], ctx.needs_input_grad[1], y, c,
-                                          2.0 / y.numel(), Sg=Sg)
+                                          2.0 / y.numel(), Sg=Sg, consumer=ctx.consumer)
         return gx, gH, None, None
 
 
@@ -1742,8 +1806,11 @@
     def float_eval(self, ctx):
         return self.float_with_grad or not (ctx.needs_input_grad[1] or ctx.needs_input_grad[2])
 
-    def lanes_grads(self, sec, gH, G, cfg, Wr=None):
+    def lanes_grads(self, sec, gH, G, cfg, Wr=None, planes=None):
         return None
+
+    def lanes_blocks(self, G, cfg, Wr=None):
+        return 0
 
 
 class RawSections(_Design, namedtuple("RawSections", "kind b a")):
@@ -1789,16 +1856,20 @@
                                                   consts.data_ptr(), b.data_ptr(), a.data_ptr(), _stream()), "geq_sections")
         return (xc, consts, b, a), geq if prologue else None
 
-    def lanes_grads(self, sec, gH, G, cfg, Wr=None):
+    def lanes_blocks(self, G, cfg, Wr=None):
         if G is None:
+            return 0
+        mode = int(Wr is not None)
+        return max(_geq_lanes_blocks(cfg, G.shape[1] if mode else 1, Wr.shape[1] if mode else 0, mode), 0)
+
+    def lanes_grads(self, sec, gH, G, cfg, Wr=None, planes=None):
+        nbx = self.lanes_blocks(G, cfg, Wr)
+        if nbx <= 0:
             return None
         mode = int(Wr is not None)
         No, Nmid, Ni = (G.shape[0], G.shape[1], Wr.shape[1]) if mode else (cfg.C, 1, 0)
-        nbx = _geq_lanes_blocks(cfg, Nmid, Ni, mode)
-        if nbx <= 0:
-            return None
         xc, consts, b, a = sec
-        out, gW = _geq_backward_lanes(mode, gH, G, b, a, Wr, cfg, No, Nmid, Ni, nbx, xc, consts, _is_sigmoid(self.gain_map))
+        out, gW = _geq_backward_lanes(mode, gH, G, b, a, Wr, cfg, No, Nmid, Ni, nbx, xc, consts, _is_sigmoid(self.gain_map), planes)
         return (out, None, gW) if mode else (out, None)
 
     def param_grads(self, sec, part, partW=None, Wr=None):
@@ -1991,7 +2062,7 @@
     return int(fn(cfg.m_local, cfg.C, cfg.S, cfg.nfft, cfg.bin0, int(ppr), int(niw), int(mode)))
 
 
-def _geq_backward_lanes(mode, gH, G, b, a, Wr, cfg, No, Nmid, Ni, nbx, xc, consts, sig):
+def _geq_backward_lanes(mode, gH, G, b, a, Wr, cfg, No, Nmid, Ni, nbx, xc, consts, sig, planes=None):
     gamma, nfft, S, C_, bin0, m_local, real = cfg
     dev = b.device
     g = _h_planar(gH.resolve_conj(), True)
@@ -2003,10 +2074,16 @@
     partW = torch.empty((Nmid * Ni, wrows), dtype=real, device=dev) if mode == 1 else None
     Wc = Wr.to(real).contiguous() if mode == 1 else None
     with kernel_timer.span("sos_response_bwd_rc" if mode == 1 else "sos_response_bwd"):
-        _lib.check(_fn("fl_geq_response_bwd_lanes", real, True)(
-            mode, g.data_ptr(), _lead_pitch(g.movedim(0, -1)), G.data_ptr(), _pitch(m_local), b.data_ptr(), a.data_ptr(), S, No, Nmid, Ni,
-            None if Wc is None else Wc.data_ptr(), gamma, twiddles(nfft, torch.float64, dev).data_ptr(), nfft, bin0, m_local,
-            psum.data_ptr(), pq.data_ptr(), None if partW is None else partW.data_ptr(), _stream()), "geq_response_bwd_lanes")
+        if planes is not None:
+            _lib.check(L.fl_geq_response_bwd_lanes_planes_c64(
+                mode, g.data_ptr(), _lead_pitch(g.movedim(0, -1)), planes.shape[0], planes.stride(0), G.data_ptr(), _pitch(m_local),
+                b.data_ptr(), a.data_ptr(), S, No, Nmid, Ni, Wc.data_ptr(), gamma, twiddles(nfft, torch.float64, dev).data_ptr(), nfft,
+                bin0, m_local, psum.data_ptr(), pq.data_ptr(), partW.data_ptr(), _stream()), "geq_response_bwd_lanes")
+        else:
+            _lib.check(_fn("fl_geq_response_bwd_lanes", real, True)(
+                mode, g.data_ptr(), _lead_pitch(g.movedim(0, -1)), G.data_ptr(), _pitch(m_local), b.data_ptr(), a.data_ptr(), S, No, Nmid,
+                Ni, None if Wc is None else Wc.data_ptr(), gamma, twiddles(nfft, torch.float64, dev).data_ptr(), nfft, bin0, m_local,
+                psum.data_ptr(), pq.data_ptr(), None if partW is None else partW.data_ptr(), _stream()), "geq_response_bwd_lanes")
     out = torch.empty_like(xc)
     gW = torch.empty(Wr.shape, dtype=real, device=dev) if mode == 1 else None
     _lib.check((L.fl_geq_sections_bwd_lanes_f64 if f64 else L.fl_geq_sections_bwd_lanes)(
@@ -2032,10 +2109,43 @@
     @staticmethod
     def backward(ctx, gH):
         *sec, G, Wr = ctx.saved_tensors
-        g = ctx.design.lanes_grads(sec, gH, G, ctx.cfg, Wr)
+        gH, planes = _gh_handoff(ctx, gH)
+        g = ctx.design.lanes_grads(sec, gH, G, ctx.cfg, Wr, planes)
         if g is None:
+            if planes is not None:
+                gH = _gh_add_planes(gH, [planes], 0)
             g = ctx.design.param_grads(sec, *_cascade_rc_backward(gH, G, *sec[2:], Wr, ctx.cfg), Wr)
         return (None, *g, None, None, None)
+
+
+def _gh_add_planes(gH, sets, first):
+    for parts in sets:
+        rest = parts[first:]
+        if rest.shape[0] > 1:
+            n = rest[0].numel()
+            tot = torch.empty_like(rest[0])
+            with kernel_timer.span("sum_parts"):
+                _lib.check(_lib.lib().fl_sum_parts_c64(rest.data_ptr(), rest.stride(0), rest.shape[0], tot.data_ptr(), n, _stream()), "sum_parts")
+        else:
+            tot = rest[0]
+        gH = gH + tot[..., :gH.shape[0]].movedim(-1, 0)
+    return gH
+
+
+def _gh_handoff(ctx, gH):
+    pending = ctx.__dict__.pop("_gh_parts", None)
+    if not pending:
+        return gH, None
+    task = _graph_task()
+    sets = [(parts, M) for t, parts, M in pending if t == task]
+    if not sets:
+        return gH, None
+    if len(sets) == 1:
+        parts, M = sets[0]
+        p0 = parts[0][..., :M].movedim(-1, 0)
+        if gH.data_ptr() == p0.data_ptr() and gH.shape == p0.shape and gH.stride() == p0.stride() and gH.dtype == p0.dtype:
+            return gH, parts
+    return _gh_add_planes(gH, [parts for parts, _ in sets], 1), None
 
 
 def sos_response_rc(b, a, Wr, gamma: float, nfft: int, dtype=torch.float32) -> torch.Tensor:
diff --git a/include/flamo_hip.h b/include/flamo_hip.h
--- a/include/flamo_hip.h
+++ b/include/flamo_hip.h
@@ -65,6 +65,11 @@
 int fl_spec_gradh_walk_f32(const void* Sg, const void* Xp, void* dH_parts, long ds_s, long ds_m, long ds_n, int n_slices, const void* W,
                            int nfft, int Bn, int NI, int NO, double scale_g, int interior2_g, const void* out_scale, void* stream);
 int fl_sum_parts_c64(const void* parts, long part_stride, int n_parts, void* out, long n, void* stream);
+int fl_spec_gradh_pieces(int nfft, int Bn, int NI, int NO, int* records, int* info);
+int fl_spec_gradh_walk_pieces_f32(const void* Sg, const void* Xp, void* dH_parts, long ds_s, long ds_m, long ds_n, const void* pieces,
+                                  int n_records, int n_planes, int nsc, const void* W, int nfft, int Bn, int NI, int NO, double scale_g,
+                                  int interior2_g, const void* out_scale, void* stream);
+int fl_debug_set_gradh_pieces(int n0, int n1, int n2);
 int fl_debug_set_walk(int mode, int wgs, int slices, void* times);
 int fl_debug_set_walk_stamps(void* buf);
 int fl_wall_clock_khz(void);
@@ -204,6 +209,10 @@
 int fl_geq_response_bwd_lanes_c64(int mode, const void* gH, long g_pitch, const void* G, long h_pitch, const void* b, const void* a,
                                   int S, int No, int Nmid, int Ni, const void* Wr, double gamma, const void* Wd, int nfft,
                                   int bin0, int m_local, void* psum, void* pq, void* partW, void* stream);
+int fl_geq_response_bwd_lanes_planes_c64(int mode, const void* gH, long g_pitch, int n_planes, long g_plane, const void* G,
+                                         long h_pitch, const void* b, const void* a, int S, int No, int Nmid, int Ni, const void* Wr,
+                                         double gamma, const void* Wd, int nfft, int bin0, int m_local, void* psum, void* pq,
+                                         void* partW, void* stream);
 int fl_geq_sections_bwd_lanes(const void* gain, int in_kind, const void* psum, const void* pq, int nbx, const void* b, const void* a,
                               double gamma, int nb, int C, const void* consts, void* ggain, const void* partW, int wrows, int wn,
                               void* gW, void* stream);
```

Result: slower. 644.1 billion products/s (-5.5%).
